# sailab-code/GNN_tf_2.x

Hardware: AMD Instinct MI355X
Metric: node-state-updates/sec (nodes x iters / s), 1M-node synthetic graph (higher is better)
Workload: dtype f32; 1 GPU; synthetic randomGraph-recipe graph, N=1000000 nodes, E=9999690 arcs, state_dim=64, net_state 135->128->128->64 selu+BN, net_output 67->2 softmax+BN, max_iter=30, threshold=0 (all iterations run); the loop-invariant label aggregates (GNN.py:259, :263; 0.2 ms) are kept between Loops until the labels change, see cold_aggregates_ms_per_step; parallelism=single GPU, tile_form=one wave per 32-node tile (k_fused)

## Files before the change

### gnn_tf_2.x_amd/GNN/_engine.py

```python
from __future__ import annotations

import ctypes as C
import os

import numpy as np

_HERE = os.path.dirname(os.path.abspath(__file__))
LIB_PATH = os.environ.get('GNN_HIP_LIBRARY') or os.path.join(_HERE, 'libgnn_hip.so')

ACT_CODES = {'linear': 0, None: 0, 'relu': 1, 'selu': 2, 'elu': 3, 'tanh': 4, 'sigmoid': 5, 'softmax': 6}

EXPORTS = ['gnn_last_error', 'gnn_version', 'gnn_device_count', 'gnn_device_synchronize', 'gnn_graph_create', 'gnn_graph_create_from_arcs',
           'gnn_graph_derive', 'gnn_graph_derive_edge', 'gnn_graph_set_arc_order', 'gnn_graph_update_labels', 'gnn_graph_get_nodes', 'gnn_graph_dims', 'gnn_graph_destroy',
           'gnn_mlp_create', 'gnn_mlp_set_weights', 'gnn_mlp_get_weights', 'gnn_mlp_reset_optimizer', 'gnn_mlp_forward', 'gnn_mlp_destroy', 'gnn_loop_create',
           'gnn_loop_set_state0', 'gnn_loop_run', 'gnn_loop_get_state', 'gnn_loop_get_output', 'gnn_loop_readout', 'gnn_loop_set_edge_readout', 'gnn_loop_train_step',
           'gnn_loop_train_forward', 'gnn_loop_train_backward', 'gnn_loop_arm_optimizer', 'gnn_loop_optimizer_step', 'gnn_loop_update_moving_statistics', 'gnn_loss_grad',
           'gnn_loss_grad_ex', 'gnn_loop_set_loss_params', 'gnn_train_forms', 'gnn_loop_train_forms', 'gnn_loop_train_mask', 'gnn_fused_net_form', 'gnn_small_form',
           'gnn_loop_set_train_persistent', 'gnn_train_persistent_form', 'gnn_loop_train_info',
           'gnn_mlp_set_regularizers', 'gnn_loop_set_clipping', 'gnn_loop_grad_sqnorm', 'gnn_loop_optimizer_step_scaled',
           'gnn_counters_get', 'gnn_lgnn_run', 'gnn_loop_run_many', 'gnn_loop_set_impl', 'gnn_loop_gate_info', 'gnn_loop_set_pieces', 'gnn_loop_range_info', 'gnn_split_f16_exponent', 'gnn_split_f16', 'gnn_loop_set_persistent', 'gnn_loop_set_tile_form', 'gnn_loop_set_gather_form', 'gnn_gather_program_build', 'gnn_graph_gather_program_info', 'gnn_loop_drop_cached_aggregates', 'gnn_loop_set_profiling', 'gnn_loop_get_timing', 'gnn_loop_get_exchange_timing', 'gnn_loop_destroy', 'gnn_shard_range',
           'gnn_comm_unique_id', 'gnn_comm_create', 'gnn_comm_allreduce_max', 'gnn_comm_destroy', 'gnn_halo_plan', 'gnn_graph_create_halo',
           'gnn_comm_create_loopback', 'gnn_graph_set_full_adjacency', 'gnn_loop_set_slice_exchange', 'gnn_loop_run_group', 'gnn_loop_readout_group', 'gnn_graph_update_labels_group']

_lib = None


class EngineError(RuntimeError):
    pass


def lib():
    global _lib
    if _lib is None:
        if not os.path.exists(LIB_PATH):
            raise EngineError(f'{LIB_PATH} is missing: build it with `python -c "import __graft_entry__ as g; g.build()"` '
                              f'or `make -C gnn_tf_2.x_amd/csrc`')
        _lib = C.CDLL(LIB_PATH)
        _lib.gnn_last_error.restype = C.c_char_p
        for name in EXPORTS:
            if name != 'gnn_last_error':
                getattr(_lib, name).restype = C.c_int
    return _lib


def loss_grad(loss_kind: int, targets, out, sample_weights, label_smoothing: float = 0.0, huber_delta: float = 1.0):
    t, o, w = _f32(targets), _f32(out), _f32(sample_weights)
    if t.shape != o.shape or w.shape != (o.shape[0],): raise ValueError(f'targets {t.shape}, outputs {o.shape}, weights {w.shape} do not match')
    d = np.zeros_like(o)
    loss = C.c_double()
    _check(lib().gnn_loss_grad_ex(C.c_int(loss_kind), C.c_int64(o.shape[0]), C.c_int(o.shape[1]), _fp(t), _fp(o), _fp(w), C.c_double(label_smoothing),
                                  C.c_double(huber_delta), C.byref(loss), _fp(d)))
    return float(loss.value), d


FORM_NAMES = {0: 'per_op', 1: 'mlp_fwd', 2: 'wide', 3: 'chain3', 4: 'wgrad_bf', 5: 'wgrad_f32'}


def _forms_dict(out):
    names = [FORM_NAMES[int(v)] for v in out[3:]]
    return dict(forward=names[0::3], backward=names[1::3], wgrad=names[2::3], build_input=bool(out[1]), sweep_rows=int(out[2]))


def train_forms(dims, activations, rates=None, n_rows=0, producer_dropout=True) -> dict:
    L = len(dims) - 1
    if L < 1 or len(activations) != L: raise ValueError('dims needs one entry more than activations')
    d = np.ascontiguousarray(dims, np.int32)
    a = np.asarray([ACT_CODES[x] for x in activations], np.int32)
    r = _f32(rates if rates is not None else np.zeros(L + 1), (L + 1,))
    out = np.zeros(3 + 3 * L, np.int32)
    _check(lib().gnn_train_forms(C.c_int(L), _ip(d), _ip(a), _fp(r), C.c_int64(int(n_rows)), C.c_int(bool(producer_dropout)), _ip(out)))
    return _forms_dict(out)


ACT_NAMES = {v: k for k, v in ACT_CODES.items() if k is not None}


def fused_net_form(dims, activations, nlc=0) -> dict:
    L = len(dims) - 1
    if L < 1 or len(activations) != L: raise ValueError('dims needs one entry more than activations')
    d = np.ascontiguousarray(dims, np.int32)
    a = np.asarray([ACT_CODES[x] for x in activations], np.int32)
    out = np.zeros(6, np.int32)
    _check(lib().gnn_fused_net_form(C.c_int(L), _ip(d), _ip(a), C.c_int(int(nlc)), _ip(out)))
    if not out[0]: return dict(covered=False, hidden=None, last=None, NT=0, NTL=0, mixed=False)
    return dict(covered=True, hidden=ACT_NAMES[int(out[1])], last=ACT_NAMES[int(out[2])], NT=int(out[3]), NTL=int(out[4]), mixed=bool(out[5]))


def small_form(dims, activations, n_rows, nlc=0) -> dict:
    L = len(dims) - 1
    if L < 1 or len(activations) != L: raise ValueError('dims needs one entry more than activations')
    d = np.ascontiguousarray(dims, np.int32)
    a = np.asarray([ACT_CODES[x] for x in activations], np.int32)
    out = np.zeros(3, np.int32)
    _check(lib().gnn_small_form(C.c_int(L), _ip(d), _ip(a), C.c_int(int(nlc)), C.c_int64(int(n_rows)), _ip(out)))
    return dict(persistent=bool(out[0]), tile=int(out[0]), wide=bool(out[1]), steps=int(out[2]))


TRAIN_PERSISTENT_MAX_BYTES = 256 << 20


def train_persistent_form(dims, activations, n_rows, max_iter, rates=None) -> dict:
    L = len(dims) - 1
    if L < 1 or len(activations) != L: raise ValueError('dims needs one entry more than activations')
    d = np.ascontiguousarray(dims, np.int32)
    a = np.asarray([ACT_CODES[x] for x in activations], np.int32)
    r = _f32(rates if rates is not None else np.zeros(L + 1), (L + 1,))
    out = np.zeros(5, np.int32)
    _check(lib().gnn_train_persistent_form(C.c_int(L), _ip(d), _ip(a), _fp(r), C.c_int64(int(n_rows)), C.c_int(int(max_iter)), _ip(out)))
    return dict(persistent=bool(out[0]), workgroups=int(out[1]), rows=int(out[2]), lds=int(out[3]), body_bytes=int(out[4]))


def split_f16(values, exponent=None):
    v = np.ascontiguousarray(values, np.float32).ravel()
    if exponent is None:
        exponent = int(lib().gnn_split_f16_exponent(C.c_float(float(np.max(np.abs(v))) if v.size else 0.0)))
    p0, p1 = np.empty(v.size, np.uint16), np.empty(v.size, np.uint16)
    lib().gnn_split_f16(v.ctypes.data_as(C.c_void_p), C.c_int(v.size), C.c_int(int(exponent)), p0.ctypes.data_as(C.c_void_p), p1.ctypes.data_as(C.c_void_p))
    return p0.view(np.float16), p1.view(np.float16), int(exponent)


def _check(rc: int):
    if rc == 0:
        return
    msg = lib().gnn_last_error().decode(errors='replace')
    if rc == -1:
        raise ValueError(msg)
    if rc == -5:
        raise NotImplementedError(msg)
    raise EngineError(f'[gnn_status {rc}] {msg}')


def _f32(a, shape=None):
    a = np.ascontiguousarray(a, dtype=np.float32)
    if shape is not None and a.shape != tuple(shape):
        raise ValueError(f'expected shape {tuple(shape)}, got {a.shape}')
    return a


def _fp(a):
    return a.ctypes.data_as(C.POINTER(C.c_float)) if a is not None else None


def _ip(a):
    return a.ctypes.data_as(C.POINTER(C.c_int32)) if a is not None else None


def device_count() -> int:
    n = C.c_int(0)
    _check(lib().gnn_device_count(C.byref(n)))
    return n.value


def require_device(device: int = 0) -> None:
    n = device_count()
    if n <= device:
        raise EngineError(f'no HIP device {device} visible ({n} found): this engine only runs on MI355X (gfx950)')


def shard_range(n_nodes: int, rank: int, world: int) -> tuple[int, int]:
    b, n = C.c_int64(0), C.c_int64(0)
    _check(lib().gnn_shard_range(C.c_int64(n_nodes), C.c_int(rank), C.c_int(world), C.byref(b), C.byref(n)))
    return b.value, n.value


def gather_program(indptr, adj_src, adj_w):
    indptr = np.ascontiguousarray(indptr, dtype=np.int32)
    adj_src = np.ascontiguousarray(adj_src, dtype=np.int32)
    adj_w = _f32(adj_w)
    n_rows = indptr.size - 1
    hdr = np.zeros((n_rows // 32, 2), np.int32)
    nb = C.c_int64(0)
    _check(lib().gnn_gather_program_build(C.c_int64(n_rows), _ip(indptr), _ip(adj_src), _fp(adj_w), _ip(hdr), None, C.byref(nb)))
    ent = np.zeros((nb.value, 64, 2), np.int32)
    _check(lib().gnn_gather_program_build(C.c_int64(n_rows), _ip(indptr), _ip(adj_src), _fp(adj_w), None, _ip(ent), C.byref(nb)))
    return hdr, ent.view(np.uint32)


def halo_plan(n_nodes: int, world: int, indptr, adj_src):
    indptr = np.ascontiguousarray(indptr, dtype=np.int32)
    adj_src = np.ascontiguousarray(adj_src, dtype=np.int32)
    slot = np.empty(n_nodes, np.int32)
    counts = np.zeros(world, np.int64)
    block = C.c_int64(0)
    _check(lib().gnn_halo_plan(C.c_int64(n_nodes), C.c_int(world), _ip(indptr), _ip(adj_src), _ip(slot),
                               counts.ctypes.data_as(C.POINTER(C.c_int64)), C.byref(block)))
    return slot, counts, int(block.value)


def shard_halo(n_nodes: int, rank: int, world: int, indptr, adj_src, nodes, plan=None):
    slot, counts, block = plan if plan is not None else halo_plan(n_nodes, world, indptr, adj_src)
    rb, nr = shard_range(n_nodes, rank, world)
    shard = ((n_nodes + world - 1) // world + 31) // 32 * 32
    indptr = np.asarray(indptr)
    e0, e1 = int(indptr[rb]), int(indptr[rb + nr])
    src = np.asarray(adj_src)[e0:e1].astype(np.int64)
    owner = src // shard
    mine = owner == rank
    if np.any(~mine & (slot[src] < 0)):
        raise ValueError('halo plan does not cover a remote source')
    remapped = np.where(mine, src - rb, shard + owner * block + slot[src]).astype(np.int32)
    nodes = np.asarray(nodes, np.float32)
    rep = np.zeros((shard + world * block, nodes.shape[1]), np.float32)
    rep[:nr] = nodes[rb:rb + nr]
    for q in range(world):
        qb, qn = shard_range(n_nodes, q, world)
        ids = qb + np.nonzero(slot[qb:qb + qn] >= 0)[0]
        rep[shard + q * block: shard + q * block + len(ids)] = nodes[ids]
    send = np.nonzero(slot[rb:rb + nr] >= 0)[0].astype(np.int32)
    return dict(block=block, send_rows=send, adj_src=remapped, nodes=rep, row_begin=rb, n_rows=nr, e0=e0, e1=e1)


def shard_csr(n_nodes: int, rank: int, world: int, indptr, *per_entry_arrays):
    rb, nr = shard_range(n_nodes, rank, world)
    indptr = np.asarray(indptr)
    e0, e1 = int(indptr[rb]), int(indptr[rb + nr])
    return (rb, nr, (indptr[rb:rb + nr + 1] - e0).astype(np.int32)) + tuple(np.asarray(a)[e0:e1] for a in per_entry_arrays)


class Graph:

    def __init__(self, n_nodes, indptr, adj_src, adj_w, arc_w, arc_labels, nodes, mask, row_begin=0, device=0, _handle=None):
        self._h = C.c_void_p()
        if _handle is not None:
            self._h = _handle
            return
        require_device(device)
        indptr = np.ascontiguousarray(indptr, dtype=np.int32)
        adj_src = np.ascontiguousarray(adj_src, dtype=np.int32)
        adj_w, arc_w = _f32(adj_w), _f32(arc_w)
        arc_labels, nodes = _f32(arc_labels), _f32(nodes)
        mask = np.ascontiguousarray(mask, dtype=np.uint8)
        n_rows, n_arcs = len(indptr) - 1, len(adj_src)
        if arc_labels.ndim != 2 or arc_labels.shape[0] != n_arcs or nodes.ndim != 2 or nodes.shape[0] != n_nodes:
            raise ValueError('arc_labels must be [n_arcs, AL] and nodes [n_nodes, NL]')
        if len(adj_w) != n_arcs or len(arc_w) != n_arcs or len(mask) != n_rows:
            raise ValueError('inconsistent array lengths')
        _check(lib().gnn_graph_create(C.c_int64(n_nodes), C.c_int64(row_begin), C.c_int64(n_rows), C.c_int64(n_arcs),
                                      _ip(indptr), _ip(adj_src), _fp(adj_w), _fp(arc_w), _fp(arc_labels),
                                      C.c_int(arc_labels.shape[1]), _fp(nodes), C.c_int(nodes.shape[1]),
                                      mask.ctypes.data_as(C.POINTER(C.c_uint8)), C.c_int(device), C.byref(self._h)))

    @classmethod
    def halo(cls, n_nodes_global, rank, world, block, send_rows, indptr, adj_src_replica, adj_w, arc_w, arc_labels, nodes_replica, mask, device=0):
        require_device(device)
        indptr = np.ascontiguousarray(indptr, dtype=np.int32)
        adj = np.ascontiguousarray(adj_src_replica, dtype=np.int32)
        send = np.ascontiguousarray(send_rows, dtype=np.int32)
        adj_w, arc_w, arc_labels, nodes_replica = _f32(adj_w), _f32(arc_w), _f32(arc_labels), _f32(nodes_replica)
        mask = np.ascontiguousarray(mask, dtype=np.uint8)
        if len(adj_w) != len(adj) or len(arc_w) != len(adj) or arc_labels.shape[0] != len(adj) or len(mask) != len(indptr) - 1:
            raise ValueError('inconsistent array lengths')
        h = C.c_void_p()
        _check(lib().gnn_graph_create_halo(C.c_int64(n_nodes_global), C.c_int(rank), C.c_int(world), C.c_int64(block), C.c_int64(len(send)), _ip(send),
                                           C.c_int64(len(adj)), _ip(indptr), _ip(adj), _fp(adj_w), _fp(arc_w), _fp(arc_labels), C.c_int(arc_labels.shape[1]),
                                           _fp(nodes_replica), C.c_int(nodes_replica.shape[1]), mask.ctypes.data_as(C.POINTER(C.c_uint8)), C.c_int(device), C.byref(h)))
        return cls(None, None, None, None, None, None, None, None, _handle=h)

    @classmethod
    def from_arcs(cls, n_nodes, arc_src, arc_dst, arc_labels, aggregation_mode, nodes, mask, device=0):
        require_device(device)
        modes = {'sum': 0, 'normalized': 1, 'average': 2}
        if aggregation_mode not in modes: raise ValueError('ERROR: Unknown aggregation mode')
        arc_src = np.ascontiguousarray(arc_src, dtype=np.int32)
        arc_dst = np.ascontiguousarray(arc_dst, dtype=np.int32)
        arc_labels, nodes = _f32(arc_labels), _f32(nodes)
        mask = np.ascontiguousarray(mask, dtype=np.uint8)
        e = len(arc_src)
        if len(arc_dst) != e or arc_labels.shape[0] != e or nodes.shape[0] != n_nodes or len(mask) != n_nodes:
            raise ValueError('inconsistent array lengths')
        indptr, adj_src, arc_id = np.zeros(n_nodes + 1, np.int32), np.zeros(e, np.int32), np.zeros(e, np.int32)
        adj_w, arc_w = np.zeros(e, np.float32), np.zeros(e, np.float32)
        h = C.c_void_p()
        _check(lib().gnn_graph_create_from_arcs(C.c_int64(n_nodes), C.c_int64(e), _ip(arc_src), _ip(arc_dst), _fp(arc_labels),
                                                C.c_int(arc_labels.shape[1]), C.c_int(modes[aggregation_mode]), _fp(nodes), C.c_int(nodes.shape[1]),
                                                mask.ctypes.data_as(C.POINTER(C.c_uint8)), C.c_int(device), C.byref(h), _ip(indptr), _ip(adj_src),
                                                _fp(adj_w), _ip(arc_id), _fp(arc_w)))
        return cls(None, None, None, None, None, None, None, None, _handle=h), indptr, adj_src, adj_w, arc_id, arc_w

    def dims(self):
        n, r, e, m = C.c_int64(), C.c_int64(), C.c_int64(), C.c_int64()
        nl, al = C.c_int(), C.c_int()
        _check(lib().gnn_graph_dims(self._h, C.byref(n), C.byref(r), C.byref(e), C.byref(nl), C.byref(al), C.byref(m)))
        return dict(n_nodes=n.value, n_rows=r.value, n_arcs=e.value, NL=nl.value, AL=al.value, n_masked=m.value)

    def derive(self, extra: int) -> 'Graph':
        h = C.c_void_p()
        _check(lib().gnn_graph_derive(self._h, C.c_int(extra), C.byref(h)))
        d = Graph(None, None, None, None, None, None, None, None, _handle=h)
        d._base = self
        return d

    def derive_edge(self, extra_nodes: int, extra_arcs: int) -> 'Graph':
        h = C.c_void_p()
        _check(lib().gnn_graph_derive_edge(self._h, C.c_int(extra_nodes), C.c_int(extra_arcs), C.byref(h)))
        d = Graph(None, None, None, None, None, None, None, None, _handle=h)
        d._base = self
        return d

    def gather_program_info(self) -> dict:
        t, b, n, ms = C.c_int64(0), C.c_int64(0), C.c_int64(0), C.c_float(0)
        _check(lib().gnn_graph_gather_program_info(self._h, C.byref(t), C.byref(b), C.byref(n), C.byref(ms)))
        return dict(tiles=t.value, batches=b.value, bytes=n.value, build_ms=ms.value)

    def set_arc_order(self, arc_id, arc_labels_orig) -> None:
        arc_id = np.ascontiguousarray(arc_id, dtype=np.int32)
        _check(lib().gnn_graph_set_arc_order(self._h, _ip(arc_id), _fp(_f32(arc_labels_orig))))

    def update_labels(self, base: 'Graph', loop: 'Loop', get_state: bool, get_output: bool) -> None:
        _check(lib().gnn_graph_update_labels(self._h, base._h, loop._h, C.c_int(bool(get_state)), C.c_int(bool(get_output))))

    def set_full_adjacency(self, n_global: int, indptr, adj_src, adj_w):
        ip, src, w = np.ascontiguousarray(indptr, np.int32), np.ascontiguousarray(adj_src, np.int32), _f32(adj_w)
        _check(lib().gnn_graph_set_full_adjacency(self._h, C.c_int64(n_global), _ip(ip), _ip(src), _fp(w)))

    @staticmethod
    def update_labels_group(dsts, bases, loops, get_state: bool, get_output: bool) -> None:
        n = len(loops)
        arr = lambda xs: (C.c_void_p * n)(*[x._h for x in xs])
        _check(lib().gnn_graph_update_labels_group(arr(dsts), arr(bases), arr(loops), C.c_int(n), C.c_int(bool(get_state)), C.c_int(bool(get_output))))

    def nodes(self) -> np.ndarray:
        d = self.dims()
        out = np.empty((d['n_nodes'], d['NL']), dtype=np.float32)
        _check(lib().gnn_graph_get_nodes(self._h, _fp(out)))
        return out

    def close(self):
        if self._h:
            lib().gnn_graph_destroy(self._h)
            self._h = C.c_void_p()

    def __del__(self):
        try:
            self.close()
        except Exception:
            pass


class Mlp:

    def __init__(self, weights, activations, batch_normalization, bn_eps=1e-3, device=0):
        require_device(device)
        self._h = C.c_void_p()
        self.n = len(activations)
        self.activations = list(activations)
        self.batch_normalization = bool(batch_normalization)
        for a in activations:
            if a not in ACT_CODES:
                raise ValueError(f'unsupported activation {a!r}')
        w, b, bn = self._pack(weights)
        self.dims = np.array([w[0].shape[0]] + [x.shape[1] for x in w], dtype=np.int32)
        acts = np.array([ACT_CODES[a] for a in activations], dtype=np.int32)
        wp = (C.POINTER(C.c_float) * self.n)(*[_fp(x) for x in w])
        bp = (C.POINTER(C.c_float) * self.n)(*[_fp(x) for x in b])
        _check(lib().gnn_mlp_create(C.c_int(self.n), _ip(self.dims), _ip(acts), wp, bp, _fp(bn), C.c_float(bn_eps),
                                    C.c_int(device), C.byref(self._h)))

    def _pack(self, weights):
        n = self.n
        if len(weights) != 2 * n + (4 if self.batch_normalization else 0):
            raise ValueError(f'expected {2 * n + (4 if self.batch_normalization else 0)} weight arrays, got {len(weights)}')
        w = [_f32(weights[2 * l]) for l in range(n)]
        b = [_f32(weights[2 * l + 1]) for l in range(n)]
        for l in range(n):
            if w[l].ndim != 2 or b[l].shape != (w[l].shape[1],) or (l and w[l].shape[0] != w[l - 1].shape[1]):
                raise ValueError(f'layer {l}: inconsistent weight shapes')
        bn = None
        if self.batch_normalization:
            bn = np.ascontiguousarray(np.concatenate([_f32(a).ravel() for a in weights[2 * n:]]))
            if bn.size != 4 * w[-1].shape[1]:
                raise ValueError('BatchNormalization arrays must each have the output width')
        return w, b, bn

    def set_weights(self, weights):
        w, b, bn = self._pack(weights)
        if [x.shape for x in w] != [(int(self.dims[l]), int(self.dims[l + 1])) for l in range(self.n)]:
            raise ValueError('weight shapes differ from the ones this MLP was created with')
        wp = (C.POINTER(C.c_float) * self.n)(*[_fp(x) for x in w])
        bp = (C.POINTER(C.c_float) * self.n)(*[_fp(x) for x in b])
        _check(lib().gnn_mlp_set_weights(self._h, wp, bp, _fp(bn)))

    def get_weights(self):
        w = [np.empty((int(self.dims[l]), int(self.dims[l + 1])), np.float32) for l in range(self.n)]
        b = [np.empty((int(self.dims[l + 1]),), np.float32) for l in range(self.n)]
        f = int(self.dims[-1])
# ... 235 lines not shown
        gs = np.zeros(sum(int(np.prod(x)) for x in shp_s), np.float32)
        go = np.zeros(sum(int(np.prod(x)) for x in shp_o), np.float32)
        bns = np.zeros((max(1, kk), 2, int(net_state.dims[-1])), np.float32)
        bno = np.zeros((2, int(net_output.dims[-1])), np.float32)
        d_out = _f32(d_out_nodes)
        if d_out.shape != (self.n_masked, self.T): raise ValueError(f'd_out_nodes shape {d_out.shape} != {(self.n_masked, self.T)}')
        dse = None
        if d_state_extra is not None:
            dse = _f32(d_state_extra)
            if dse.shape != (self.n_rows, self.Ds): raise ValueError(f'd_state_extra shape {dse.shape} != {(self.n_rows, self.Ds)}')
        dims = self.graph.dims()
        dn = np.zeros((self.n_rows, dims['NL']), np.float32) if want_d_nodes else None
        da = np.zeros((dims['n_arcs'], dims['AL']), np.float32) if want_d_arcs else None
        _check(lib().gnn_loop_train_backward(self._h, _fp(d_out), _fp(dse), _fp(gs), _fp(go), _fp(bns), _fp(bno), _fp(dn), _fp(da)))

        def split(flat, shp):
            out, off = [], 0
            for x in shp:
                cnt = int(np.prod(x))
                out.append(flat[off:off + cnt].reshape(x).copy())
                off += cnt
            return out

        return dict(grads_state=split(gs, shp_s), grads_output=split(go, shp_o), bn_batch_state=bns[:kk], bn_batch_output=bno, d_nodes=dn, d_arcs=da)

    def train_forms(self, net: int = 0) -> dict:
        out = np.zeros(3 + 3 * self._keep[1 + net].n, np.int32)
        _check(lib().gnn_loop_train_forms(self._h, C.c_int(net), _ip(out)))
        return _forms_dict(out)

    def train_mask(self, net: int, body: int, pos: int) -> np.ndarray:
        count = C.c_int64()
        _check(lib().gnn_loop_train_mask(self._h, C.c_int(net), C.c_int(body), C.c_int(pos), None, C.byref(count)))
        width = int(self._keep[1 + net].dims[pos])
        out = np.zeros(count.value, np.uint8)
        _check(lib().gnn_loop_train_mask(self._h, C.c_int(net), C.c_int(body), C.c_int(pos), out.ctypes.data_as(C.POINTER(C.c_uint8)), C.byref(count)))
        return out.reshape(-1, width).astype(bool)

    def set_impl(self, impl: int) -> int:
        used = C.c_int(0)
        _check(lib().gnn_loop_set_impl(self._h, C.c_int(impl), C.byref(used)))
        return used.value

    def gate_info(self) -> tuple:
        a, b = C.c_int(0), C.c_int(0)
        _check(lib().gnn_loop_gate_info(self._h, C.byref(a), C.byref(b)))
        return bool(a.value), int(b.value)

    def set_pieces(self, pieces: int) -> int:
        used = C.c_int(0)
        _check(lib().gnn_loop_set_pieces(self._h, C.c_int(int(pieces)), C.byref(used)))
        return used.value

    def range_info(self) -> tuple:
        a, b = C.c_int(0), C.c_int(0)
        _check(lib().gnn_loop_range_info(self._h, C.byref(a), C.byref(b)))
        return bool(a.value), int(b.value)

    def set_persistent(self, enable: bool) -> bool:
        used = C.c_int(0)
        _check(lib().gnn_loop_set_persistent(self._h, C.c_int(bool(enable)), C.byref(used)))
        return bool(used.value)

    def set_train_persistent(self, enable: bool) -> bool:
        used = C.c_int(0)
        _check(lib().gnn_loop_set_train_persistent(self._h, C.c_int(bool(enable)), C.byref(used)))
        return bool(used.value)

    def train_info(self) -> dict:
        out = np.zeros(4, np.int32)
        _check(lib().gnn_loop_train_info(self._h, _ip(out)))
        return dict(persistent=bool(out[0]), workgroups=int(out[1]), barriers_per_body=int(out[2]), timeouts=int(out[3]))

    def set_tile_form(self, form: int) -> int:
        used = C.c_int(0)
        _check(lib().gnn_loop_set_tile_form(self._h, C.c_int(int(form)), C.byref(used)))
        return used.value

    def set_gather_form(self, form: int) -> int:
        used = C.c_int(0)
        _check(lib().gnn_loop_set_gather_form(self._h, C.c_int(int(form)), C.byref(used)))
        return used.value

    def counters(self) -> dict:
        b, f, it, tot, avg = C.c_double(), C.c_double(), C.c_int(), C.c_float(), C.c_float()
        _check(lib().gnn_counters_get(self._h, C.byref(b), C.byref(f), C.byref(it), C.byref(tot), C.byref(avg)))
        return dict(bytes_per_iteration=b.value, flops_per_iteration=f.value, iterations=it.value, total_ms=tot.value, avg_iteration_ms=avg.value)

    @staticmethod
    def lgnn_run(loops, graphs, get_state: bool, get_output: bool) -> list:
        n = len(loops)
        ks = (C.c_float * n)()
        _check(lib().gnn_lgnn_run((C.c_void_p * n)(*[x._h for x in loops]), (C.c_void_p * n)(*[x._h for x in graphs]), C.c_int(n),
                                  C.c_int(bool(get_state)), C.c_int(bool(get_output)), ks))
        return [float(k) for k in ks]

    def drop_cached_aggregates(self):
        _check(lib().gnn_loop_drop_cached_aggregates(self._h))

    def set_profiling(self, on: bool):
        _check(lib().gnn_loop_set_profiling(self._h, C.c_int(bool(on))))

    def run(self, training: bool = False) -> float:
        k = C.c_float(0)
        _check(lib().gnn_loop_run(self._h, C.c_int(bool(training)), C.byref(k)))
        return float(k.value)

    @staticmethod
    def run_many(loops) -> list:
        n = len(loops)
        hs = (C.c_void_p * n)(*[l._h for l in loops])
        ks = (C.c_float * n)()
        _check(lib().gnn_loop_run_many(hs, C.c_int(n), ks))
        return [float(x) for x in ks]

    @staticmethod
    def run_group(loops) -> float:
        n = len(loops)
        hs = (C.c_void_p * n)(*[l._h for l in loops])
        k = C.c_float(0)
        _check(lib().gnn_loop_run_group(hs, C.c_int(n), C.byref(k)))
        return float(k.value)

    @staticmethod
    def readout_group(loops, ng_indptr, ng_node, ng_w) -> np.ndarray:
        n = len(loops)
        hs = (C.c_void_p * n)(*[l._h for l in loops])
        ng_indptr = np.ascontiguousarray(ng_indptr, dtype=np.int32)
        ng_node = np.ascontiguousarray(ng_node, dtype=np.int32)
        ng_w = _f32(ng_w)
        g = len(ng_indptr) - 1
        out = np.empty((g, loops[0].T), dtype=np.float32)
        _check(lib().gnn_loop_readout_group(hs, C.c_int(n), C.c_int(g), _ip(ng_indptr), _ip(ng_node), _fp(ng_w), _fp(out)))
        return out

    def timing(self):
        tot, avg, n = C.c_float(), C.c_float(), C.c_int()
        _check(lib().gnn_loop_get_timing(self._h, C.byref(tot), C.byref(avg), C.byref(n)))
        gap = C.c_float()
        _check(lib().gnn_loop_get_exchange_timing(self._h, C.byref(gap)))
        return dict(total_ms=tot.value, avg_iter_ms=avg.value, n_iter_timed=n.value, avg_between_bodies_ms=gap.value)

    def state(self) -> np.ndarray:
        out = np.empty((self.n_rows, self.Ds), dtype=np.float32)
        _check(lib().gnn_loop_get_state(self._h, _fp(out)))
        return out

    def output(self) -> np.ndarray:
        out = np.empty((self.n_masked, self.T), dtype=np.float32)
        m = C.c_int64(0)
        _check(lib().gnn_loop_get_output(self._h, _fp(out), C.byref(m)))
        return out

    def readout(self, ng_indptr, ng_node, ng_w) -> np.ndarray:
        ng_indptr = np.ascontiguousarray(ng_indptr, dtype=np.int32)
        ng_node = np.ascontiguousarray(ng_node, dtype=np.int32)
        ng_w = _f32(ng_w)
        g = len(ng_indptr) - 1
        out = np.empty((g, self.T), dtype=np.float32)
        _check(lib().gnn_loop_readout(self._h, C.c_int(g), _ip(ng_indptr), _ip(ng_node), _fp(ng_w), _fp(out)))
        return out

    def close(self):
        if self._h:
            lib().gnn_loop_destroy(self._h)
            self._h = C.c_void_p()
# ... 7 lines not shown
```

### gnn_tf_2.x_amd/csrc/gnn_build.hip

```cpp
#include <hipcub/hipcub.hpp>
#include <string.h>

#include <algorithm>
#include <chrono>
#include <new>
#include <vector>

#include "gnn_common.h"
#include "gnn_fused.h"

namespace {

inline unsigned cdiv(int64_t a, int64_t b) { return (unsigned)((a + b - 1) / b); }

__global__ void k_keys(int64_t e, const int32_t *src, const int32_t *dst, unsigned long long *key, int32_t *id, int32_t *indeg)
{
    const int64_t a = (int64_t)blockIdx.x * blockDim.x + threadIdx.x;
    if (a >= e) return;
    key[a] = ((unsigned long long)(uint32_t)dst[a] << 32) | (uint32_t)src[a];
    id[a] = (int32_t)a;
    atomicAdd(indeg + dst[a], 1);
}

__global__ void k_values(int64_t e, const int32_t *dst, const int32_t *indeg, int mode, float *w)
// ... 152 lines not shown
        if (adj_w_out) HIPCHK_G(hipMemcpy(adj_w_out, sh->adj_w, sizeof(float) * E, hipMemcpyDeviceToHost));
        if (arc_id_out) HIPCHK_G(hipMemcpy(arc_id_out, d_perm2, sizeof(int32_t) * E, hipMemcpyDeviceToHost));
        if (arc_w_out) HIPCHK_G(hipMemcpy(arc_w_out, sh->arc_w, sizeof(float) * E, hipMemcpyDeviceToHost));
    }
    *out = g;
    return GNN_OK;
#undef HIPCHK_G
}

namespace {

void gather_program_split(const int (&slots)[32], int (&start)[5], int &longest)
{
    int lo = 0, hi = 0;
    for (int r = 0; r < 32; ++r) { lo = std::max(lo, slots[r]); hi += slots[r]; }
    auto groups_needed = [&](int cap) {
        int n = 1, fill = 0;
        for (int r = 0; r < 32; ++r) {
            if (fill + slots[r] > cap) { ++n; fill = 0; }
            fill += slots[r];
        }
        return n;
    };
    while (lo < hi) {
        const int mid = lo + (hi - lo) / 2;
        if (groups_needed(mid) <= 4) hi = mid; else lo = mid + 1;
    }
    int g = 0, fill = 0;
    start[0] = 0;
    for (int r = 0; r < 32; ++r) {
        if (fill + slots[r] > lo) { start[++g] = r; fill = 0; }
        fill += slots[r];
    }
    while (g < 4) start[++g] = 32;
    longest = lo;
}

}

extern "C" int gnn_gather_program_build(int64_t n_rows, const int32_t *indptr, const int32_t *adj_src, const float *adj_w, int32_t *hdr,
                                        int32_t *ent, int64_t *n_batches)
{
    ARGCHK(n_rows >= 0 && indptr && n_batches, "n_rows / indptr / n_batches are required");
    const int64_t tiles = n_rows / 32;
    ARGCHK(indptr[tiles * 32] == 0 || (adj_src && adj_w), "arc arrays are required");
    int64_t batch = 0;
    for (int64_t t = 0; t < tiles; ++t) {
        const int32_t *ip = indptr + t * 32;
        int slots[32], start[5], longest = 0;
        for (int r = 0; r < 32; ++r) {
            ARGCHK(ip[r + 1] >= ip[r], "indptr not monotone at row %lld", (long long)(t * 32 + r));
            slots[r] = std::max(1, ip[r + 1] - ip[r]);
        }
        gather_program_split(slots, start, longest);
        const int nb = (longest + 15) / 16;
        ARGCHK(batch + nb < ((int64_t)1 << 31) / 64, "gather program too large");
        if (hdr) { hdr[2 * t] = (int32_t)batch; hdr[2 * t + 1] = nb; }
        if (ent) {
            for (int g = 0; g < 4; ++g) {
                int s = 0;
                auto put = [&](uint32_t word, float w) {
                    int32_t *e = ent + (((batch + s / 16) * 64 + 16 * g + s % 16) * 2);
                    memcpy(e, &word, 4);
                    memcpy(e + 1, &w, 4);
                    ++s;
                };
                for (int r = start[g]; r < start[g + 1]; ++r) {
                    if (ip[r + 1] == ip[r]) put(GNN_GP_NOROW | GNN_GP_ROW_END | (uint32_t)r, 0.0f);
                    for (int32_t e = ip[r]; e < ip[r + 1]; ++e) {
                        if (adj_src[e] < 0 || adj_src[e] >= (1 << 23))
                            return gnn_fail(GNN_ERR_UNSUPPORTED, "adj_src[%d]=%d does not fit a gather-program source word", e, adj_src[e]);
                        put((uint32_t)adj_src[e] << 8 | (e + 1 == ip[r + 1] ? GNN_GP_ROW_END : 0u) | (uint32_t)r, adj_w[e]);
                    }
                }
                while (s < 16 * nb) put(GNN_GP_NOROW, 0.0f);
            }
        }
        batch += nb;
    }
    *n_batches = batch;
    return GNN_OK;
}

int gnn_gather_program_ensure(const gnn_graph *g)
{
    gnn_graph_shared *sh = g->sh;
    if (sh->gp_tried) return GNN_OK;
    sh->gp_tried = true;
    const int64_t tiles = g->n_rows / 32, rem = g->n_rows % 32;
    if (tiles == 0) return GNN_OK;
    int dev_before = -1;
    if (hipGetDevice(&dev_before) != hipSuccess || hipSetDevice(g->device) != hipSuccess) { (void)hipGetLastError(); return GNN_OK; }
    const auto t0 = std::chrono::steady_clock::now();
    int32_t *d_hdr = nullptr, *d_ent = nullptr;
    int64_t batches = 0, last_batches = 0;
    int32_t last_hdr[2] = {0, 0};
    bool ok = false;
    try {
        std::vector<int32_t> indptr((size_t)g->n_rows + 1), hdr((size_t)tiles * 2), src, ent;
        std::vector<float> w;
        ok = hipMemcpy(indptr.data(), sh->indptr, sizeof(int32_t) * indptr.size(), hipMemcpyDeviceToHost) == hipSuccess;
        const size_t E = ok ? (size_t)indptr.back() : 0;
        if (rem) indptr.resize((size_t)(tiles + 1) * 32 + 1, indptr.back());
        src.resize(E); w.resize(E);
        ok = ok && (E == 0 || (hipMemcpy(src.data(), sh->adj_src, sizeof(int32_t) * E, hipMemcpyDeviceToHost) == hipSuccess &&
                               hipMemcpy(w.data(), sh->adj_w, sizeof(float) * E, hipMemcpyDeviceToHost) == hipSuccess));
        for (size_t e = 0; ok && e < E; ++e) ok = src[e] >= 0 && src[e] < (1 << 23);
        const int32_t *last_ip = indptr.data() + tiles * 32;
        ok = ok && gnn_gather_program_build(tiles * 32, indptr.data(), src.data(), w.data(), hdr.data(), nullptr, &batches) == GNN_OK;
        if (ok && rem) ok = gnn_gather_program_build(32, last_ip, src.data(), w.data(), last_hdr, nullptr, &last_batches) == GNN_OK;
        ok = ok && batches + last_batches < ((int64_t)1 << 31) / 64;
        if (ok) {
            ent.resize((size_t)(batches + last_batches) * 128);
            ok = gnn_gather_program_build(tiles * 32, indptr.data(), src.data(), w.data(), nullptr, ent.data(), &batches) == GNN_OK;
            if (ok && rem) ok = gnn_gather_program_build(32, last_ip, src.data(), w.data(), nullptr, ent.data() + (size_t)batches * 128, &last_batches) == GNN_OK;
        }
        ok = ok && gnn_dev_malloc((void **)&d_hdr, sizeof(int32_t) * hdr.size()) == hipSuccess &&
             gnn_dev_malloc((void **)&d_ent, sizeof(int32_t) * ent.size()) == hipSuccess &&
             hipMemcpy(d_hdr, hdr.data(), sizeof(int32_t) * hdr.size(), hipMemcpyHostToDevice) == hipSuccess &&
             hipMemcpy(d_ent, ent.data(), sizeof(int32_t) * ent.size(), hipMemcpyHostToDevice) == hipSuccess;
    } catch (const std::bad_alloc &) { ok = false; }
    if (ok) {
        sh->gp_hdr = d_hdr; sh->gp_ent = d_ent; sh->gp_tiles = tiles; sh->gp_batches = batches + last_batches;
        sh->gp_rows = g->n_rows; sh->gp_last_first = (int32_t)batches; sh->gp_last_nb = (int32_t)last_batches;
        sh->gp_build_ms = std::chrono::duration<float, std::milli>(std::chrono::steady_clock::now() - t0).count();
    } else {
        (void)hipFree(d_hdr); (void)hipFree(d_ent);
        (void)hipGetLastError();
    }
    (void)hipSetDevice(dev_before);
    return GNN_OK;
}

extern "C" int gnn_graph_gather_program_info(const gnn_graph *g, int64_t *tiles, int64_t *batches, int64_t *bytes, float *build_ms)
{
    ARGCHK(g, "graph is NULL");
    const gnn_graph_shared *sh = g->sh;
    const bool have = sh->gp_ent != nullptr;
    if (tiles) *tiles = have ? sh->gp_tiles : 0;
    if (batches) *batches = have ? sh->gp_batches : 0;
    if (bytes) *bytes = have ? sh->gp_tiles * 8 + sh->gp_batches * 512 : 0;
    if (build_ms) *build_ms = have ? sh->gp_build_ms : 0.0f;
    return GNN_OK;
}
```

### gnn_tf_2.x_amd/csrc/gnn_common.h

```cpp
#pragma once
#include <hip/hip_runtime.h>
#include <stdint.h>
#include <string>
#include <vector>

#include "gnn_hip.h"
#include "gnn_fused.h"

int gnn_fail(int code, const char *fmt, ...);

hipError_t gnn_dev_malloc(void **p, size_t bytes);
bool gnn_poison_enabled();

inline hipError_t gnn_raise_dynamic_lds(const void *const *kernels, int n, size_t bytes, bool (&raised)[64])
{
    int dev = 0;
    hipError_t e = hipGetDevice(&dev);
    if (e != hipSuccess) return e;
    const bool listed = dev >= 0 && dev < 64;
    if (listed && raised[dev]) return hipSuccess;
    for (int i = 0; i < n && e == hipSuccess; ++i) e = hipFuncSetAttribute(kernels[i], hipFuncAttributeMaxDynamicSharedMemorySize, (int)bytes);
    if (listed && e == hipSuccess) raised[dev] = true;
    return e;
}
// ... 53 lines not shown
#define GNN_FLAG_WORDS (GNN_FLAG_SLOTS * GNN_FLAG_STRIDE)
#define GNN_BODY_CHUNK 16
#define GNN_BODY_LOOKAHEAD 4

__device__ __forceinline__ bool gnn_gate_open(const int *gate, int world)
{
    if (!gate) return true;
    int any = 0;
    for (int p = 0; p < world * GNN_FLAG_SLOTS; ++p) any |= gate[p * GNN_FLAG_STRIDE];
    return any != 0;
}

__device__ __forceinline__ bool gnn_gate_open_block(const int *gate, int world)
{
    if (!gate) return true;
    __shared__ int gate_any;
    if (threadIdx.x == 0) gate_any = 0;
    __syncthreads();
    int any = 0;
    for (int p = threadIdx.x; p < world * GNN_FLAG_SLOTS; p += blockDim.x) any |= gate[p * GNN_FLAG_STRIDE];
    if (any) gate_any = 1;
    __syncthreads();
    return gate_any != 0;
}

__device__ __forceinline__ void gnn_flag_raise(int *flag_rank_base)
{
    int *w = flag_rank_base + (blockIdx.x & (GNN_FLAG_SLOTS - 1)) * GNN_FLAG_STRIDE;
    if (__hip_atomic_load(w, __ATOMIC_RELAXED, __HIP_MEMORY_SCOPE_AGENT) == 0) atomicOr(w, 1);
}

#define GNN_BAND_ABS 1e-5f
#define GNN_BAND_REL 1e-3f
__device__ __forceinline__ bool gnn_gate_borderline(float root, float rhs, float band) { return band > 0.0f && __builtin_fabsf(root - rhs) <= band; }
struct GnnFlagPeek { int c0, c1, c2; };
__device__ __forceinline__ GnnFlagPeek gnn_flag_peek(int *flag_rank_base)
{
    int *w = flag_rank_base + (blockIdx.x & (GNN_FLAG_SLOTS - 1)) * GNN_FLAG_STRIDE;
    GnnFlagPeek p;
    p.c0 = __hip_atomic_load(w, __ATOMIC_RELAXED, __HIP_MEMORY_SCOPE_AGENT);
    p.c1 = __hip_atomic_load(w + 1, __ATOMIC_RELAXED, __HIP_MEMORY_SCOPE_AGENT);
    p.c2 = __hip_atomic_load(w + 2, __ATOMIC_RELAXED, __HIP_MEMORY_SCOPE_AGENT);
    return p;
}
__device__ __forceinline__ void gnn_flag_raise_peeked(int *flag_rank_base, const GnnFlagPeek &p, bool moved, bool robust, bool border)
{
    int *w = flag_rank_base + (blockIdx.x & (GNN_FLAG_SLOTS - 1)) * GNN_FLAG_STRIDE;
    if (moved && p.c0 == 0) atomicOr(w, 1);
    if (robust && p.c1 == 0) atomicOr(w + 1, 1);
    if (border && p.c2 == 0) atomicOr(w + 2, 1);
}

__device__ __forceinline__ void gnn_flag_raise_certified(int *flag_rank_base, bool moved, bool robust, bool border)
{
    int *w = flag_rank_base + (blockIdx.x & (GNN_FLAG_SLOTS - 1)) * GNN_FLAG_STRIDE;
    if (!(moved || border)) return;
    const int c0 = __hip_atomic_load(w, __ATOMIC_RELAXED, __HIP_MEMORY_SCOPE_AGENT);
    const int c1 = __hip_atomic_load(w + 1, __ATOMIC_RELAXED, __HIP_MEMORY_SCOPE_AGENT);
    const int c2 = __hip_atomic_load(w + 2, __ATOMIC_RELAXED, __HIP_MEMORY_SCOPE_AGENT);
    if (moved && c0 == 0) atomicOr(w, 1);
    if (robust && c1 == 0) atomicOr(w + 1, 1);
    if (border && c2 == 0) atomicOr(w + 2, 1);
}

struct gnn_graph_shared {
    int refs = 1;
    int32_t *indptr = nullptr, *adj_src = nullptr, *masked_rows = nullptr;
    float *adj_w = nullptr, *arc_w = nullptr, *arc_labels = nullptr;
    uint8_t *mask = nullptr;
    int max_degree = 0;
    int32_t *src_indptr = nullptr, *src_dst = nullptr;
    float *src_w = nullptr;
    int32_t *arc_id = nullptr;
    float *arc_labels_orig = nullptr;
    int32_t *full_indptr = nullptr, *full_src = nullptr;
    float *full_w = nullptr;
    int64_t full_rows = 0;
    int32_t *gp_hdr = nullptr, *gp_ent = nullptr;
    int64_t gp_tiles = 0, gp_batches = 0;
    int64_t gp_rows = 0;
    int32_t gp_last_first = 0, gp_last_nb = 0;
    bool gp_tried = false;
    float gp_build_ms = 0.0f;
};

struct gnn_graph {
    int device = 0;
    int64_t N = 0, N_global = 0, row_begin = 0, own_off = 0, n_rows = 0, E = 0, n_masked = 0;
    int NL = 0, AL = 0;
    int halo_world = 0, halo_rank = 0;
    int64_t halo_block = 0, halo_count = 0;
    int32_t *halo_send = nullptr;
    bool halo_send_owned = true;
    int64_t nodes_rows = 0;
    gnn_graph_shared *sh = nullptr;
    float *nodes = nullptr;
    int base_NL = 0;
    float *arc_labels_own = nullptr, *arc_labels_orig_own = nullptr;
    int base_AL = 0;
    uint64_t label_version = 1;
    hipEvent_t ready = nullptr;
};

inline const float *gnn_graph_arc_labels(const gnn_graph *g) { return g->arc_labels_own ? g->arc_labels_own : g->sh->arc_labels; }

struct gnn_mlp {
    int device = 0;
    int n_layers = 0;
    std::vector<int> dims, acts;
    std::vector<float *> W, b;
    float *slab = nullptr;
    size_t slab_floats = 0;
    float *bn_scale = nullptr, *bn_shift = nullptr;
    float *bn_raw = nullptr;
    float *opt_a = nullptr, *opt_b = nullptr;
    float *opt_c = nullptr;
    int opt_kind = -1;
    std::vector<double> reg_l1, reg_l2;
    bool has_bn = false;
    float eps = 1e-3f;
    float *packed = nullptr;
    size_t packed_floats = 0;
    int *packed_split = nullptr;
    size_t packed_split_dwords = 0;
    int split_exp[3] = {0, 0, 0};
    int pack_nlc = -1;
    bool pack_dirty = true;
    uint64_t version = 0;
};

struct gnn_loop;
struct gnn_comm_group {
    int world = 1, refs = 0;
    hipStream_t stream = nullptr;
    std::vector<gnn_loop *> member;
};

struct gnn_comm {
    int rank = 0, world = 1, device = 0;
    void *nccl = nullptr;
    gnn_comm_group *grp = nullptr;
    hipStream_t stream = nullptr;
    hipStream_t xstream = nullptr;
    double *scratch = nullptr;
    int loops = 0;
    bool closed = false;
};

struct gnn_train_settings {
    struct { bool armed = false; int kind = 0; float h[4] = {0, 0, 0, 0}; bool mean = false; float mom_s = 0.99f, mom_o = 0.99f; } opt;
    struct { float value = 0.0f; double norm = 0.0, global = 0.0; } clip;
    struct { double smoothing = 0.0, delta = 1.0; } loss;
    struct { bool allowed = false, failed = false; int timeouts = 0; } persistent;
    int k_hint = 0;
};
#define GNN_INTERNAL __attribute__((visibility("hidden")))
struct GNN_INTERNAL gnn_train_ctx;
struct GNN_INTERNAL gnn_train_arena;

struct gnn_loop {
    gnn_graph *g = nullptr;
    gnn_mlp *st = nullptr, *ou = nullptr;
    gnn_comm *comm = nullptr;
    int device = 0, rank = 0, world = 1;
    int D = 0, Ds = 0, NLc = 0, in_s = 0, wf = 0, T = 0, max_iter = 0;
    float thr = 0.f;
    int64_t shard_rows = 0, N_pad = 0, own_off = 0;
    hipStream_t stream = nullptr;
    float *state[2] = {nullptr, nullptr};
    float *state_init = nullptr;
    bool init_in_place = false;
    float *inp = nullptr;
    float *inv = nullptr;
    uint64_t inv_version = 0;
    bool inv_zeroed = false;
    float *tmp[2] = {nullptr, nullptr};
    float *feats = nullptr, *out = nullptr, *otmp[2] = {nullptr, nullptr};
    int *flags = nullptr;
    int *tile_ctr = nullptr;
    int *kfinal_dev = nullptr, *kfinal_host = nullptr;
    int certified_reruns = 0;
    bool last_run_rerun = false;
    int pieces = 2;
    int range_reruns = 0;
    bool last_run_range_rerun = false;
    bool small_words_clean = false;
    unsigned small_runs = 0;
    float *small_xs = nullptr;
    size_t small_xs_floats = 0;
    bool small_disabled = false;
    int kfinal = -1;
    bool have_state0 = false, ran = false;
    bool graph_ready_seen = false;
    int impl_req = 1;
    int tile_form = 0;
    int gather_form = 0;
    LoopForm form;
    int32_t *ng_ip = nullptr, *ng_node = nullptr;
    float *ng_w = nullptr, *ng_out = nullptr, *ng_part = nullptr;
    std::vector<int32_t> ng_key;
    std::vector<float> ng_w_host;
    float *ng_host = nullptr;
    int ng_G = 0, ng_host_floats = 0;
    bool ng_inlaunch = false;
    uint64_t out_runs = 0, ng_inlaunch_run = 0;
    bool edge_mode = false, edge_expected = false;
    int32_t *edge_dst = nullptr, *edge_rows = nullptr;
    float *edge_labels = nullptr;
    int64_t n_edge_masked = 0;
    int32_t *edge_inc_ptr = nullptr, *edge_inc = nullptr;
    int *gate_host = nullptr;
    hipEvent_t ev_gate = nullptr;
    bool profiling = false;
    std::vector<hipEvent_t> ev;
    hipEvent_t ev_total[2] = {nullptr, nullptr};
    float total_ms = 0.f, avg_iter_ms = 0.f;
    float avg_gap_ms = 0.f;
    int n_iter_timed = 0;
    bool slice_mode = false;
    int Cs = 0;
    float *sl_send = nullptr;
    float *sl_state = nullptr;
    float *sl_agg = nullptr;
    float *sl_recv = nullptr;
    bool sl_pipeline = true;
    std::vector<hipEvent_t> sl_ev;
    hipEvent_t sl_done = nullptr;
    float *agg_own = nullptr;
    gnn_train_ctx *train_ctx = nullptr;
    gnn_train_arena *train_arena = nullptr;
    gnn_train_settings train;
};

inline bool gnn_loop_ng_folded(const gnn_loop *l) { return l->ng_inlaunch && l->ng_inlaunch_run == l->out_runs; }

int gnn_graph_wait_ready(const gnn_graph *g, hipStream_t st);
int gnn_launch_spmm(hipStream_t st, int64_t n_rows, const int32_t *indptr, const int32_t *idx, const float *w, const float *X,
                    int width, int64_t ldx, float *out, int64_t ldo, const int *gate, int world);
int gnn_launch_dense(hipStream_t st, int64_t n, int n_in, int n_out, const float *X, int64_t ldx, const float *W, const float *b,
                     int act, float *Y, int64_t ldy);
int gnn_launch_check(hipStream_t st, int64_t n_rows, int d, const float *s, const float *so, float thr, int *flag_rank_base);
int gnn_comm_allgather32(gnn_comm *c, const void *send, void *recv, size_t count, hipStream_t st);
int gnn_launch_feats_edge(hipStream_t st, const gnn_loop *l, const float *state, float *feats);
int gnn_launch_copy_cols(hipStream_t st, int64_t n_rows, int w, const float *src, int64_t lds_, float *dst, int64_t ldd, const int *gate, int world);
int gnn_mlp_refresh_bn(gnn_mlp *m, hipStream_t st);
void gnn_train_ctx_free(gnn_loop *l);
void gnn_train_arena_free(gnn_loop *l);

int gnn_loop_decide_form(gnn_loop *l);
inline int gnn_loop_impl_used(const gnn_loop *l) { return l->form.path == GNN_PATH_UNFUSED ? 0 : (l->form.split ? 2 : 1); }
int gnn_gather_program_ensure(const gnn_graph *g);
int gnn_fused_prepare(gnn_loop *l);
int gnn_fused_pack(gnn_mlp *m, int nlc);
int gnn_fused_iteration(gnn_loop *l, int k);
int gnn_small_run(gnn_loop *l);
void gnn_fused_release(gnn_mlp *m);
```

### gnn_tf_2.x_amd/csrc/gnn_fused.h

```cpp
#pragma once
#include <hip/hip_runtime.h>
#include <stdint.h>

constexpr int GNN_FUSED_MAXL = 3;
constexpr int GNN_FUSED_WAVES = 8;
constexpr int GNN_FUSED_THREADS = 64 * GNN_FUSED_WAVES;
#define GNN_F16_EX 4
#define GNN_F16_LIMIT 65504.0f
#define GNN_GP_ROW_MASK 31u
#define GNN_GP_ROW_END 32u
#define GNN_GP_NOROW 0xfffffe00u
constexpr int GNN_ACTL_FROM_ARGS = -1;

struct GnnFusedArgs {
    int64_t n_rows, row_begin;
    const int32_t *indptr, *adj_src;
    const float *adj_w;
    const float *inv;
    const float *state_cur;
    float *state_nxt;
    int64_t state_bytes;
    int Ds, NLc, AL, IW, in_s, c_aggs, KP, lpr, lpr_log2, vec, kk0;
    const float *Wp[GNN_FUSED_MAXL];
    const float *bias[GNN_FUSED_MAXL];
    const float *bn_scale, *bn_shift;
    float thr;
    const int *gate;
    int *flag_out;
    int world;
    int certify;
    int *tile_ctr;
    int wstride;
    int stagger;
    const int *Ws[GNN_FUSED_MAXL];
    int chunks0;
    int pieces;
    float bsc[GNN_FUSED_MAXL], usc[GNN_FUSED_MAXL];
    const int *Ws_base;
    int ws_bytes, ws_off[GNN_FUSED_MAXL];
    int tile_base;
    int full_tiles;
    int variant;
    const float *agg_in;
    const int32_t *gp_hdr, *gp_ent;
    int gp_tiles, gp_last_first, gp_last_nb;
    int threads;
    int single_ticket;
    unsigned long long *stamps;
    int lds_floats;
    int act_last;
};

struct GnnSmallCtl {
    float *state0, *state1;
    const float *init;
    int *kfinal;
    int *flags;
    int *host_result;
    float *xs;
    int DP;
    int rnd;
    const float *Wraw[GNN_FUSED_MAXL];
    int din[GNN_FUSED_MAXL], dout[GNN_FUSED_MAXL];
    int KP16;
    int *zero_words;
    int n_words;
    int max_iter;
    float *out;
    const uint8_t *mask;
    const int32_t *mask_pos;
    const float *nodes_own;
    const float *ow, *ob, *obn_scale, *obn_shift;
    int NL, NLc, T, oact;
    const int32_t *ng_ip, *ng_node;
    const float *ng_w;
    float *ng_host;
    int G, ro_word;
    int ecache;
};

struct FusedPlan {
    int layers = 0, NT = 0, NTL = 0, KP = 0, kk0 = 0;
    int act = 0, act_last = 0;
    int pad = 0, KPs = 0;
    int nt[GNN_FUSED_MAXL] = {0, 0, 0};
    int kk[GNN_FUSED_MAXL] = {0, 0, 0};
    size_t w_off[GNN_FUSED_MAXL] = {0, 0, 0}, b_off[GNN_FUSED_MAXL] = {0, 0, 0}, bn_off = 0, total = 0;
    int chunks[GNN_FUSED_MAXL] = {0, 0, 0};
    size_t s_off[GNN_FUSED_MAXL] = {0, 0, 0}, h_off[GNN_FUSED_MAXL] = {0, 0, 0}, s_total = 0;
};

enum GnnLoopPath { GNN_PATH_UNFUSED = 0, GNN_PATH_BODIES = 1, GNN_PATH_PERSISTENT = 2 };
enum GnnBodyKernel { GNN_BODY_GENERIC = 0, GNN_BODY_FULL_TILE = 1, GNN_BODY_PAIR = 2 };
struct LoopForm {
    int path = GNN_PATH_UNFUSED;
    int kernel = GNN_BODY_GENERIC;
    bool split = false;
    int pieces = 3;
    bool program = false;
    FusedPlan plan;
    unsigned grid = 0;
    size_t lds = 0;
    GnnFusedArgs args;
    int small_tile = 0, kk_small = 0, s0 = 0;
    bool small_wide = false;
    bool fold_output = false, fold_readout = false;
    GnnSmallCtl ctl;
};

constexpr int GNN_SMALL_ECACHE = 1024;
constexpr int GNN_SMALL16_HP = 36;
constexpr int GNN_SMALL16W_HP = 66;
template <int ROWS, bool WIDE = false>
struct GnnSmallLds {
    static_assert(ROWS == 16 || ROWS == 32, "16- or 32-node tiles");
    static_assert(!WIDE || ROWS == 16, "the wide form works on 16-node tiles");
    static constexpr int H = 0;
    static constexpr int IPT = ROWS == 16 ? 16 * (WIDE ? GNN_SMALL16W_HP : GNN_SMALL16_HP) : 32;
    static constexpr int EP = IPT + ROWS + 4;
    static constexpr int HBW = WIDE ? 64 : 32;
    static constexpr int HB = EP + 96;
    static constexpr int HW = HB + 2 * HBW;
    static constexpr int SCR = HW + 544;
    static constexpr int LABELS = 32 * ROWS;
    static constexpr int EC_SRC = SCR + 2 * LABELS;
    static constexpr int EC_W = EC_SRC + GNN_SMALL_ECACHE;
    static constexpr int END = EC_W + GNN_SMALL_ECACHE + 4;
    static constexpr size_t bytes(int KP) { return sizeof(float) * ((size_t)ROWS * KP + END); }
};

template <int... V> struct GnnSteps { static constexpr int values[] = {V...}; };
using GnnSmallKK0 = GnnSteps<8, 12, 16, 24, 32, 36, 40, 48>;
using GnnSmall16S0 = GnnSteps<4, 8, 12, 16, 20, 24>;

bool gnn_small_launch(int layers, int act, int kk0, const GnnFusedArgs &a, const GnnSmallCtl &c, unsigned grid, size_t lds_bytes,
                      hipStream_t st);
bool gnn_small16_launch(int layers, int act, int s0, const GnnFusedArgs &a, const GnnSmallCtl &c, unsigned grid, size_t lds_bytes, hipStream_t st);
bool gnn_small_launch_mixed(int layers, int act, int kk0, const GnnFusedArgs &a, const GnnSmallCtl &c, unsigned grid, size_t lds_bytes,
                            hipStream_t st);
bool gnn_small16_launch_mixed(int layers, int act, int s0, const GnnFusedArgs &a, const GnnSmallCtl &c, unsigned grid, size_t lds_bytes, hipStream_t st);
bool gnn_small16w_launch(int layers, int act, int s0, const GnnFusedArgs &a, const GnnSmallCtl &c, unsigned grid, size_t lds_bytes, hipStream_t st);
bool gnn_small16w_launch_mixed(int layers, int act, int s0, const GnnFusedArgs &a, const GnnSmallCtl &c, unsigned grid, size_t lds_bytes, hipStream_t st);

bool gnn_fused_launch_l1(int act, int nt, int ntl, const GnnFusedArgs &a, unsigned grid, size_t lds_bytes, hipStream_t st);
bool gnn_fused_launch_s1(int act, int nt, int ntl, const GnnFusedArgs &a, unsigned grid, size_t lds_bytes, hipStream_t st);
bool gnn_fused_launch_s2(int act, int nt, int ntl, const GnnFusedArgs &a, unsigned grid, size_t lds_bytes, hipStream_t st);
bool gnn_fused_launch_s3(int act, int nt, int ntl, const GnnFusedArgs &a, unsigned grid, size_t lds_bytes, hipStream_t st);
bool gnn_fused_launch_p2(int act, const GnnFusedArgs &a, unsigned grid, size_t lds_bytes, hipStream_t st);
bool gnn_fused_launch_p3(int act, const GnnFusedArgs &a, unsigned grid, size_t lds_bytes, hipStream_t st);
bool gnn_fused_launch_l2(int act, int nt, int ntl, const GnnFusedArgs &a, unsigned grid, size_t lds_bytes, hipStream_t st);
bool gnn_fused_launch_l3(int act, int nt, int ntl, const GnnFusedArgs &a, unsigned grid, size_t lds_bytes, hipStream_t st);
bool gnn_fused_launch_ml2(int act, int nt, int ntl, const GnnFusedArgs &a, unsigned grid, size_t lds_bytes, hipStream_t st);
bool gnn_fused_launch_ml3(int act, int nt, int ntl, const GnnFusedArgs &a, unsigned grid, size_t lds_bytes, hipStream_t st);
bool gnn_fused_launch_ms2(int act, int nt, int ntl, const GnnFusedArgs &a, unsigned grid, size_t lds_bytes, hipStream_t st);
bool gnn_fused_launch_ms3(int act, int nt, int ntl, const GnnFusedArgs &a, unsigned grid, size_t lds_bytes, hipStream_t st);
```

### gnn_tf_2.x_amd/csrc/gnn_fused.hip

```cpp
#include <stdio.h>
#include <stdlib.h>
#include <string.h>

#include <algorithm>
#include <cmath>
#include <vector>

#include "gnn_engine.h"
#include "gnn_fused.h"

namespace {

constexpr int MAXL = GNN_FUSED_MAXL;
constexpr int K_GROUP = 12;
constexpr int K_SLACK = 8;

constexpr int GNN_FUSED_VARIANT_DEFAULT = 1;
constexpr int GNN_FUSED_SPREAD_DEFAULT = 8;
constexpr int GNN_FUSED_SPREAD_SMALL_DEFAULT = 6;
#ifndef GNN_GATHER_FORM_DEFAULT
#define GNN_GATHER_FORM_DEFAULT 2
#endif
constexpr int S_SLACK = 2;

int round_tiles(int width) { return width <= 32 ? 1 : (width <= 64 ? 2 : 4); }

bool make_plan(const gnn_mlp *m, int nlc, FusedPlan &p)
{
    if (m->n_layers < 1 || m->n_layers > MAXL) return false;
    p.layers = m->n_layers;
    p.act_last = m->acts[m->n_layers - 1];
    p.act = m->n_layers > 1 ? m->acts[0] : p.act_last;
    int hid = 0;
    for (int l = 0; l < m->n_layers; ++l) {
        if (m->acts[l] < GNN_ACT_LINEAR || m->acts[l] >= GNN_ACT_SOFTMAX) return false;
        if (l < m->n_layers - 1 && m->acts[l] != p.act) return false;
        if (m->dims[l + 1] > 128) return false;
        if (l < m->n_layers - 1) hid = std::max(hid, m->dims[l + 1]);
    }
    p.NTL = round_tiles(m->dims.back());
    if (p.layers == 1) {
        p.NT = p.NTL;
    } else {
        p.NT = std::max(round_tiles(hid), p.NTL);
        if (p.NT > 1 && p.NTL == 1) p.NTL = 2;
    }
    p.kk0 = ((m->dims[0] + 1) / 2 + K_GROUP - 1) / K_GROUP * K_GROUP;
    p.KP = std::max(2 * p.kk0, (m->dims[0] + 15) / 16 * 16) + 1;
    size_t off = 0;
    for (int l = 0; l < p.layers; ++l) {
        p.nt[l] = l == p.layers - 1 ? p.NTL : p.NT;
        p.kk[l] = l == 0 ? p.kk0 : 16 * p.NT;
        p.w_off[l] = off;
        off += (size_t)(p.kk[l] + (l == 0 ? K_SLACK : 0)) * 64 * p.nt[l];
    }
    for (int l = 0; l < p.layers; ++l) { p.b_off[l] = off; off += 32 * (size_t)p.nt[l]; }
    p.bn_off = off;
    off += 2 * 32 * (size_t)p.NTL;
    p.total = off;
    const int ds = m->dims.back();
    p.pad = ds == 64 ? (4 - (ds + nlc) % 4) % 4 : 0;
    p.KPs = p.KP;
    if (ds == 64) {
        p.KPs = (std::max(2 * p.kk0, (m->dims[0] + p.pad + 15) / 16 * 16) + 3) / 4 * 4;
        if ((p.KPs / 4) % 2 == 0) p.KPs += 4;
    }
    size_t soff = 0;
    for (int l = 0; l < p.layers; ++l) {
        p.chunks[l] = l == 0 ? (m->dims[0] + p.pad + 15) / 16 : 2 * p.NT;
        p.s_off[l] = soff;
        soff += (size_t)(p.chunks[l] + (l == 0 ? S_SLACK : 0)) * p.nt[l] * 3 * 256;
    }
    for (int l = 0; l < p.layers; ++l) {
        p.h_off[l] = soff;
        soff += (size_t)(p.chunks[l] + (l == 0 ? S_SLACK : 0)) * p.nt[l] * 2 * 256;
    }
    p.s_total = soff;
    return true;
}

size_t lds_bytes(const FusedPlan &p)
{
    return (size_t)GNN_FUSED_WAVES * 32 * std::max(p.KP, p.KPs) * sizeof(float) + 128 + GNN_FUSED_WAVES * 36 * sizeof(int) + (3 + 2) * 32 * 4 * sizeof(float) + 16;
}

constexpr int PAIR_CH0 = 9;
bool pair_covers(const FusedPlan &p, int ds)
{
    return ds == 64 && p.NTL == 2 && p.NT == 4 && (p.layers == 2 || p.layers == 3) && p.chunks[0] == PAIR_CH0 && p.act_last == p.act;
}
int pair_xs(const FusedPlan &p)
{
    int xs = 16 * p.chunks[0] - 64 + 4;
    if ((xs / 4) % 2 == 0) xs += 4;
    return xs;
}
size_t pair_lds_bytes(const FusedPlan &p)
{
    return sizeof(float) * ((size_t)4 * (32 * pair_xs(p) + p.chunks[0] * 768) + 16 + GNN_FUSED_WAVES * 20 + 3 * 32 * 2 + 2 * 32 * 4) + 128;
}
struct SmallForm {
    int tile = 0;
    bool wide = false;
    int steps = 0;
// ... 243 lines not shown
    a.KP = split ? p.KPs : p.KP; a.kk0 = p.kk0;
    a.vec = (l->Ds % 4 == 0) ? 4 : 1;
    int lpr = 1, lg = 0;
    while ((lpr * a.vec < l->Ds || lpr < 2) && lpr < 64) { lpr <<= 1; ++lg; }
    a.lpr = lpr; a.lpr_log2 = lg;
    for (int i = 0; i < p.layers; ++i) {
        a.Wp[i] = m->packed + p.w_off[i];
        a.bias[i] = m->packed + p.b_off[i];
    }
    for (int i = 0; i < p.layers; ++i) a.Ws[i] = m->packed_split + p.s_off[i];
    a.chunks0 = p.chunks[0];
    a.Ws_base = m->packed_split;
    a.ws_bytes = (int)(p.s_total * sizeof(uint32_t));
    a.pieces = l->pieces == 2 ? 2 : 3;
    for (int i = 0; i < p.layers; ++i) {
        a.ws_off[i] = (int)((a.pieces == 2 ? p.h_off[i] : p.s_off[i]) * sizeof(uint32_t));
        const int e = a.pieces == 2 ? m->split_exp[i] + GNN_F16_EX : 0;
        a.bsc[i] = std::ldexp(1.0f, e);
        a.usc[i] = std::ldexp(1.0f, -e);
    }
    a.variant = GNN_FUSED_VARIANT_DEFAULT;
    a.bn_scale = m->has_bn ? m->packed + p.bn_off : nullptr;
    a.bn_shift = m->has_bn ? m->packed + p.bn_off + 32 * p.NTL : nullptr;
    a.thr = l->thr;
    a.world = l->world;
    a.certify = split ? 1 : 0;
    a.agg_in = l->slice_mode ? l->agg_own : nullptr;
    a.wstride = 1;
    a.act_last = p.act_last;
}

static void body_args(const gnn_loop *l, int k, GnnFusedArgs &a)
{
    const int cur = k & 1, P = l->world;
    a.state_cur = gnn_loop_state_after(l, k, 0);
    a.state_nxt = l->state[cur ^ 1] + (size_t)l->own_off * l->Ds;
    a.gate = l->flags + (size_t)k * P * GNN_FLAG_WORDS;
    a.flag_out = l->flags + ((size_t)(k + 1) * P + l->rank) * GNN_FLAG_WORDS;
    a.tile_ctr = l->tile_ctr + k;
}

static void decide_bodies(const gnn_loop *l, LoopForm &f, int n_cu)
{
    const gnn_graph *g = l->g;
    const FusedPlan &p = f.plan;
    GnnFusedArgs &a = f.args;
    fill_args(l, p, f.split, a);
    const size_t n_tiles = (size_t)((g->n_rows + 31) / 32);
#ifdef GNN_DIAG
    static const int variant_env = getenv("GNN_FUSED_VARIANT") ? atoi(getenv("GNN_FUSED_VARIANT")) : GNN_FUSED_VARIANT_DEFAULT;
    a.variant = variant_env;
    static const int debug = getenv("GNN_FUSED_DEBUG") ? atoi(getenv("GNN_FUSED_DEBUG")) : 0;
    a.wstride = (debug & 1) ? 0 : 1;
#endif
    const unsigned grid = (unsigned)std::min<size_t>((size_t)n_cu, n_tiles);
    int stagger_rounds = GNN_FUSED_SPREAD_DEFAULT;
#ifdef GNN_DIAG
    static const int stagger_env = getenv("GNN_FUSED_STAGGER") ? atoi(getenv("GNN_FUSED_STAGGER")) : GNN_FUSED_SPREAD_DEFAULT;
    stagger_rounds = stagger_env;
#endif
    a.stagger = n_tiles >= (size_t)4 * GNN_FUSED_WAVES * grid ? stagger_rounds : (n_tiles > (size_t)GNN_FUSED_WAVES * grid ? GNN_FUSED_SPREAD_SMALL_DEFAULT : 0);
#ifdef GNN_DIAG
    static const int stagger_small = getenv("GNN_FUSED_STAGGER_SMALL") ? atoi(getenv("GNN_FUSED_STAGGER_SMALL")) : 0;
    const bool small_grid = n_tiles > (size_t)GNN_FUSED_WAVES * grid && n_tiles < (size_t)4 * GNN_FUSED_WAVES * grid;
    if (small_grid && stagger_small > 0) { a.stagger = stagger_small; a.variant |= 4; }
    static const int spread_small = getenv("GNN_FUSED_SPREAD_SMALL") ? atoi(getenv("GNN_FUSED_SPREAD_SMALL")) : -1;
    if (small_grid && spread_small >= 0) a.stagger = spread_small;
#endif
    a.single_ticket = n_tiles <= (size_t)GNN_FUSED_WAVES * grid ? 1 : 0;
    f.grid = grid;
    f.lds = lds_bytes(p);
    if (f.kernel == GNN_BODY_PAIR) {
        const int64_t n_tiles64 = (int64_t)n_tiles;
        a.KP = pair_xs(p);
        a.full_tiles = 1;
        f.grid = (unsigned)std::min<int64_t>((int64_t)n_cu, (n_tiles64 + 3) / 4);
        a.stagger = n_tiles64 >= (int64_t)4 * 4 * f.grid ? stagger_rounds : (n_tiles64 > (int64_t)4 * f.grid ? GNN_FUSED_SPREAD_SMALL_DEFAULT : 0);
        f.lds = pair_lds_bytes(p);
    } else if (f.kernel == GNN_BODY_FULL_TILE) {
        a.full_tiles = 1;
        if (f.program) {
            a.gp_hdr = g->sh->gp_hdr; a.gp_ent = g->sh->gp_ent; a.gp_tiles = (int)g->sh->gp_tiles;
            a.gp_last_first = g->sh->gp_last_first; a.gp_last_nb = g->sh->gp_last_nb;
        }
    }
    a.lds_floats = gnn_poison_enabled() ? (int)(f.lds / sizeof(float)) : 0;
}

static int decide_persistent(gnn_loop *l, LoopForm &f, const SmallForm &sf)
{
    const gnn_graph *g = l->g;
    const FusedPlan &p = f.plan;
    GnnFusedArgs &a = f.args;
    fill_args(l, p, false, a);
    a.state_cur = l->state[0];
    a.state_nxt = l->state[1] + (size_t)l->own_off * l->Ds;
    GnnSmallCtl &c = f.ctl;
    c.state0 = l->state[0]; c.state1 = l->state[1];
    c.init = l->D ? l->state_init : g->nodes + (size_t)g->own_off * g->NL;
    c.kfinal = l->kfinal_dev;
    c.host_result = l->kfinal_host;
    bool tile16 = sf.tile == 16;
    f.small_wide = sf.wide;
    if (tile16) f.s0 = sf.steps; else f.kk_small = sf.steps;
#ifdef GNN_DIAG
    static const int tile_env = getenv("GNN_SMALL_TILE") ? atoi(getenv("GNN_SMALL_TILE")) : 0;
    if (tile_env == 32 && !sf.wide) {
        tile16 = false;
        f.kk_small = small_form(l->st, p, 16 * 256 + 1).steps;
    }
#endif
    f.small_tile = tile16 ? 16 : 32;
    f.grid = (unsigned)((g->n_rows + f.small_tile - 1) / f.small_tile);
    c.DP = l->Ds <= 16 ? 16 : 32;
    {
        const size_t need = (size_t)2 * f.grid * f.small_tile * c.DP;
        if (l->small_xs_floats < need) {
            if (l->small_xs) (void)hipFree(l->small_xs);
            l->small_xs = nullptr; l->small_xs_floats = 0;
            HIPCHK(gnn_dev_malloc((void **)&l->small_xs, need * sizeof(float)));
            l->small_xs_floats = need;
        }
        c.xs = l->small_xs;
    }
    c.max_iter = l->max_iter;
    c.ecache = GNN_SMALL_ECACHE;
#ifdef GNN_DIAG
    static const int ecache_env = getenv("GNN_SMALL_ECACHE") ? atoi(getenv("GNN_SMALL_ECACHE")) : GNN_SMALL_ECACHE;
    c.ecache = std::min(GNN_SMALL_ECACHE, ecache_env);
#endif
    c.n_words = (int)(((size_t)l->max_iter + 3 + 3) & ~(size_t)3);
    const gnn_mlp *ou = l->ou;
    if (!l->edge_mode && g->n_masked && ou->n_layers == 1 && l->T <= 8 && l->Ds + l->NLc <= 64 && l->Ds <= 32 && g->NL <= 32) {
        c.out = l->out; c.mask = g->sh->mask; c.mask_pos = g->sh->masked_rows + g->n_masked;
        c.nodes_own = g->nodes + (size_t)g->own_off * g->NL;
        c.ow = ou->W[0]; c.ob = ou->b[0];
        c.obn_scale = ou->has_bn ? ou->bn_scale : nullptr; c.obn_shift = ou->has_bn ? ou->bn_shift : nullptr;
        c.NL = g->NL; c.NLc = l->NLc; c.T = l->T; c.oact = ou->acts[0];
        f.fold_output = true;
        if (l->ng_ip && l->ng_G > 0 && g->n_masked == g->n_rows) {
            if (l->ng_host_floats < l->ng_G * l->T) {
                if (l->ng_host) (void)hipHostFree(l->ng_host);
                l->ng_host = nullptr; l->ng_host_floats = 0;
                if (hipHostMalloc((void **)&l->ng_host, sizeof(float) * (size_t)l->ng_G * l->T) == hipSuccess) l->ng_host_floats = l->ng_G * l->T;
            }
            if (l->ng_host) {
                c.ng_ip = l->ng_ip; c.ng_node = l->ng_node; c.ng_w = l->ng_w; c.ng_host = l->ng_host; c.G = l->ng_G; c.ro_word = l->max_iter + 1;
                f.fold_readout = true;
            }
        }
    }
    c.rnd = g->sh->max_degree > 8 ? 8 : 4;
    if (tile16) {
        const gnn_mlp *m = l->st;
        for (int q = 0; q < p.layers; ++q) { c.Wraw[q] = m->W[q]; c.din[q] = m->dims[q]; c.dout[q] = m->dims[q + 1]; }
        c.KP16 = std::max((a.in_s + 3) / 4 * 4, 4 * f.s0);
        if (c.KP16 % 8 == 0) c.KP16 += 4;
        f.lds = sf.wide ? GnnSmallLds<16, true>::bytes(c.KP16) : GnnSmallLds<16>::bytes(c.KP16);
    } else
        f.lds = GnnSmallLds<32>::bytes(p.KP);
    a.lds_floats = gnn_poison_enabled() ? (int)(f.lds / sizeof(float)) : 0;
    return GNN_OK;
}

int gnn_loop_decide_form(gnn_loop *l)
{
    LoopForm &f = l->form;
    f = LoopForm{};
    if (l->impl_req < 1) return GNN_OK;
    HIPCHK(hipSetDevice(l->device));
    if (!gnn_fused_supported(l, f.plan)) return GNN_OK;
    if (l->device < 0 || l->device >= 64) return gnn_fail(GNN_ERR_ARG, "device %d out of range", l->device);
    const gnn_graph *g = l->g;
    const FusedPlan &p = f.plan;
    const int n_cu = device_cus(l->device);
    const int64_t n_tiles = (g->n_rows + 31) / 32;
    f.split = l->impl_req == 2;
    f.pieces = l->pieces == 2 ? 2 : 3;
    const bool pair = f.split && !l->slice_mode && pair_covers(p, l->Ds) && pair_lds_bytes(p) <= 160 * 1024 &&
                      (l->tile_form ? l->tile_form == 2 : n_tiles <= (int64_t)4 * n_cu);
    f.kernel = pair ? GNN_BODY_PAIR : (l->Ds == 64 && p.NTL == 2 ? GNN_BODY_FULL_TILE : GNN_BODY_GENERIC);
    if (f.kernel == GNN_BODY_FULL_TILE && !l->slice_mode && (l->gather_form ? l->gather_form : GNN_GATHER_FORM_DEFAULT) == 2 &&
        gnn_gather_program_ensure(g) == GNN_OK)
        f.program = g->sh->gp_ent != nullptr && g->sh->gp_rows == g->n_rows;
    const SmallForm sf = small_form(l->st, p, g->n_rows);
    const bool persistent = l->world == 1 && !l->small_disabled && !l->profiling && sf.tile != 0;
    f.path = persistent ? GNN_PATH_PERSISTENT : GNN_PATH_BODIES;
    if (!l->inv) HIPCHK(gnn_dev_malloc((void **)&l->inv, inv_floats(l) * sizeof(float)));
    if (persistent) return decide_persistent(l, f, sf);
    decide_bodies(l, f, n_cu);
    return GNN_OK;
}

static bool launch_body(const LoopForm &f, const GnnFusedArgs &a, hipStream_t st)
{
    const FusedPlan &p = f.plan;
    if (p.act_last != p.act) {
        if (f.kernel == GNN_BODY_PAIR || p.layers < 2) return false;
        if (f.split) return p.layers == 2 ? gnn_fused_launch_ms2(p.act, p.NT, p.NTL, a, f.grid, f.lds, st) : gnn_fused_launch_ms3(p.act, p.NT, p.NTL, a, f.grid, f.lds, st);
        return p.layers == 2 ? gnn_fused_launch_ml2(p.act, p.NT, p.NTL, a, f.grid, f.lds, st) : gnn_fused_launch_ml3(p.act, p.NT, p.NTL, a, f.grid, f.lds, st);
    }
    if (f.kernel == GNN_BODY_PAIR)
        return p.layers == 2 ? gnn_fused_launch_p2(p.act, a, f.grid, f.lds, st) : gnn_fused_launch_p3(p.act, a, f.grid, f.lds, st);
    if (f.split) {
        if (p.layers == 1) return gnn_fused_launch_s1(p.act, p.NT, p.NTL, a, f.grid, f.lds, st);
        if (p.layers == 2) return gnn_fused_launch_s2(p.act, p.NT, p.NTL, a, f.grid, f.lds, st);
        return gnn_fused_launch_s3(p.act, p.NT, p.NTL, a, f.grid, f.lds, st);
    }
    if (p.layers == 1) return gnn_fused_launch_l1(p.act, p.NT, p.NTL, a, f.grid, f.lds, st);
    if (p.layers == 2) return gnn_fused_launch_l2(p.act, p.NT, p.NTL, a, f.grid, f.lds, st);
    return gnn_fused_launch_l3(p.act, p.NT, p.NTL, a, f.grid, f.lds, st);
}

int gnn_fused_iteration(gnn_loop *l, int k)
{
    const LoopForm &f = l->form;
    GnnFusedArgs a = f.args;
    body_args(l, k, a);
#ifdef GNN_DIAG
    static const char *stamp_file = getenv("GNN_FUSED_STAMPS");
    static unsigned long long *stamp_buf = nullptr;
    const size_t n_waves = (size_t)((l->g->n_rows + 31) / 32);
    if (stamp_file && k == 1) {
        if (!stamp_buf) HIPCHK(gnn_dev_malloc((void **)&stamp_buf, n_waves * 16 * sizeof(unsigned long long)));
        HIPCHK(hipMemsetAsync(stamp_buf, 0, n_waves * 16 * sizeof(unsigned long long), l->stream));
        a.stamps = stamp_buf;
    }
#endif
    const FusedPlan &p = f.plan;
    if (!launch_body(f, a, l->stream))
        return gnn_fail(GNN_ERR_UNSUPPORTED, "no fused instantiation for %d layers, tiles (%d,%d), activations %d / %d", p.layers, p.NT, p.NTL, p.act, p.act_last);
#ifdef GNN_DIAG
    if (a.stamps) {
        std::vector<unsigned long long> host(n_waves * (f.kernel == GNN_BODY_PAIR ? 16 : 8));
        HIPCHK(hipStreamSynchronize(l->stream));
        HIPCHK(hipMemcpy(host.data(), stamp_buf, host.size() * sizeof(unsigned long long), hipMemcpyDeviceToHost));
        if (FILE *f_ = fopen(stamp_file, "wb")) { fwrite(host.data(), sizeof(unsigned long long), host.size(), f_); fclose(f_); }
    }
#endif
    HIPCHK(hipGetLastError());
    return GNN_OK;
}

int gnn_small_run(gnn_loop *l)
{
    const LoopForm &f = l->form;
    const FusedPlan &p = f.plan;
    GnnFusedArgs a = f.args;
    GnnSmallCtl c = f.ctl;
    const size_t n_words = (size_t)c.n_words;
    l->kfinal_host[1] = 0;
    if (!l->small_words_clean) {
        HIPCHK(hipMemsetAsync(l->flags, 0, sizeof(int) * 2 * n_words, l->stream));
        l->small_words_clean = true;
        l->small_runs = 0;
    }
    c.flags = l->flags + (l->small_runs & 1) * n_words;
    c.zero_words = l->flags + ((l->small_runs & 1) ^ 1) * n_words;
    ++l->small_runs;
    l->ng_inlaunch = f.fold_readout;
    if (f.fold_readout) l->ng_inlaunch_run = l->out_runs;
#ifdef GNN_DIAG
    static const char *small_stamp_file = getenv("GNN_SMALL_STAMPS");
    static unsigned long long *small_stamp_buf = nullptr;
    if (small_stamp_file) {
        if (!small_stamp_buf) HIPCHK(gnn_dev_malloc((void **)&small_stamp_buf, 256 * sizeof(unsigned long long)));
        HIPCHK(hipMemsetAsync(small_stamp_buf, 0, 256 * sizeof(unsigned long long), l->stream));
// ... 26 lines not shown
```

### gnn_tf_2.x_amd/csrc/gnn_fused_kernel.h

```cpp
#pragma once
#include <utility>

#include "gnn_common.h"
#include "gnn_fused.h"

typedef float f32x16 __attribute__((ext_vector_type(16)));

namespace gnn_fused_dev {

#define GNN_GLOBAL __attribute__((address_space(1)))
template <class T>
__device__ __forceinline__ const GNN_GLOBAL T *gptr(const T *p) { return (const GNN_GLOBAL T *)p; }
template <class T>
__device__ __forceinline__ GNN_GLOBAL T *gptr_w(T *p) { return (GNN_GLOBAL T *)p; }
typedef float v4f __attribute__((ext_vector_type(4)));
typedef float v2f __attribute__((ext_vector_type(2)));
typedef int v4i_ __attribute__((ext_vector_type(4)));
__device__ __forceinline__ v4f gload4(const float *p) { return *(const GNN_GLOBAL v4f *)p; }
#ifndef GNN_STORE_AUX
#define GNN_STORE_AUX 2
#endif
__device__ __forceinline__ void gstore_row4(float *base, int64_t off, v4f v)
{
#if GNN_STORE_AUX == 0
// ... 811 lines not shown
    if constexpr (!PADDED) zero_pad_columns(a, X, lane, KP);
    __builtin_amdgcn_fence(__ATOMIC_ACQ_REL, "wavefront");

    int node = grp * 8;
    const int node_end = node + 8;
    const int e_begin = ipt[node], e_end = ipt[node_end];
    int next_end = ipt[node + 1];
    v2f acc01 = {0.f, 0.f}, acc23 = {0.f, 0.f};
    const __amdgpu_buffer_rsrc_t rsrc = __builtin_amdgcn_make_buffer_rsrc(const_cast<float *>(a.state_cur), 0, (int)a.state_bytes, 0x00020000);
    const int voff0 = gl * 16;
    float *xo = X + c_aggs + gl * 4;
#define GNN_ROW_BOUNDARY(e)                                                                     \
    while ((e) >= next_end) {                                                                   \
        float *xr = xo + node * KP;                                                             \
        if constexpr (AL16) *reinterpret_cast<v4f *>(xr) = v4f{acc01.x, acc01.y, acc23.x, acc23.y};   \
        else { xr[0] = acc01.x; xr[1] = acc01.y; xr[2] = acc23.x; xr[3] = acc23.y; }            \
        acc01 = v2f{0.f, 0.f}; acc23 = v2f{0.f, 0.f};                                           \
        ++node;                                                                                 \
        next_end = ipt[node + 1];                                                               \
    }
    int base = e_begin;
    for (; base + GB <= e_end; base += GB) {
        float w[GB];
        v4f x[GB];
        gather_batch<GB>(my_src, my_w, rsrc, voff0, w, x, std::make_integer_sequence<int, GB>{});
        const int nb = base + GB + gl;
        my_src = 0; my_w = 0.0f;
        if (nb < e_end) { my_src = gstream1(a.adj_src + nb); my_w = gstream1(a.adj_w + nb); }
#pragma unroll
        for (int u = 0; u < GB; ++u) {
            GNN_ROW_BOUNDARY(base + u)
            gather_fma(acc01, acc23, w[u], x[u]);
        }
    }
    {
        const int cnt = e_end - base;
        float w[GB];
        v4f x[GB];
        gather_batch<GB>(my_src, my_w, rsrc, voff0, w, x, std::make_integer_sequence<int, GB>{});
#pragma unroll
        for (int u = 0; u < GB; ++u) {
            if (u < cnt) {
                GNN_ROW_BOUNDARY(base + u)
                gather_fma(acc01, acc23, w[u], x[u]);
            }
        }
    }
#undef GNN_ROW_BOUNDARY
    for (; node < node_end; ++node) {
        float *xr = xo + node * KP;
        if constexpr (AL16) *reinterpret_cast<v4f *>(xr) = v4f{acc01.x, acc01.y, acc23.x, acc23.y};
        else { xr[0] = acc01.x; xr[1] = acc01.y; xr[2] = acc23.x; xr[3] = acc23.y; }
        acc01 = v2f{0.f, 0.f}; acc23 = v2f{0.f, 0.f};
    }
    own.write(a, X, i0, lane, KP, c_aggs);
}

template <bool AL16, int J>
__device__ __forceinline__ void prog_consume(int words, float w, v4f x, v2f &acc01, v2f &acc23, float *xo, int KP)
{
    gather_fma(acc01, acc23, w, x);
    const unsigned t = (unsigned)row_bcast_i<J>(words);
    if (t & GNN_GP_ROW_END) {
        float *xr = xo + __umul24(t & GNN_GP_ROW_MASK, (unsigned)KP);
        if constexpr (AL16) *reinterpret_cast<v4f *>(xr) = v4f{acc01.x, acc01.y, acc23.x, acc23.y};
        else { xr[0] = acc01.x; xr[1] = acc01.y; xr[2] = acc23.x; xr[3] = acc23.y; }
        acc01 = v2f{0.f, 0.f}; acc23 = v2f{0.f, 0.f};
    }
}
template <bool AL16, int GB, int... J>
__device__ __forceinline__ void prog_batch(int words, float my_w, __amdgpu_buffer_rsrc_t rsrc, int voff0, float (&w)[GB], v4f (&x)[GB],
                                           std::integer_sequence<int, J...>)
{
    ((w[J] = row_bcast_f<J>(my_w),
      x[J] = __builtin_bit_cast(v4f, __builtin_amdgcn_raw_buffer_load_b128(rsrc, (row_bcast_i<J>(words) & ~0xff) | voff0, 0, 0))), ...);
}
template <bool AL16, int GB, int... J>
__device__ __forceinline__ void prog_consume_all(int words, const float (&w)[GB], const v4f (&x)[GB], v2f &acc01, v2f &acc23, float *xo, int KP,
                                                 std::integer_sequence<int, J...>)
{
    (prog_consume<AL16, J>(words, w[J], x[J], acc01, acc23, xo, KP), ...);
}
typedef int v2i __attribute__((ext_vector_type(2)));
__device__ __forceinline__ v2i prog_header_request(const GnnFusedArgs &a, int tile)
{
    v2i h = {a.gp_last_first, tile == a.gp_tiles ? a.gp_last_nb : 0};
    if (tile < a.gp_tiles) h = *reinterpret_cast<const GNN_GLOBAL v2i *>(gptr(a.gp_hdr) + 2 * (int64_t)tile);
    return h;
}
__device__ __forceinline__ v2i prog_entry(const GnnFusedArgs &a, int b, int lane)
{
    return *reinterpret_cast<const GNN_GLOBAL v2i *>(gptr(a.gp_ent) + ((int64_t)b * 64 + lane) * 2);
}
template <bool AL16>
__device__ __forceinline__ void load_tile_prog64(const GnnFusedArgs &a, float *X, int64_t i0, int lane, int KP, int c_aggs, int first, int nb, v2i ent)
{
    constexpr int GB = 16;
    const int gl = lane & 15;
    TileOwn64<AL16> own;
    own.request(a, i0, lane);
    v2f acc01 = {0.f, 0.f}, acc23 = {0.f, 0.f};
    const __amdgpu_buffer_rsrc_t rsrc = __builtin_amdgcn_make_buffer_rsrc(const_cast<float *>(a.state_cur), 0, (int)a.state_bytes, 0x00020000);
    const int voff0 = gl * 16;
    float *xo = X + c_aggs + gl * 4;
    for (int b = 0; b < nb; ++b) {
        float w[GB];
        v4f x[GB];
        const int words = ent.x;
        prog_batch<AL16, GB>(words, __int_as_float(ent.y), rsrc, voff0, w, x, std::make_integer_sequence<int, GB>{});
        if (b + 1 < nb) ent = prog_entry(a, first + b + 1, lane);
        prog_consume_all<AL16, GB>(words, w, x, acc01, acc23, xo, KP, std::make_integer_sequence<int, GB>{});
    }
    own.write(a, X, i0, lane, KP, c_aggs);
}

#ifndef GNN_FIRST_BATCH_AHEAD
#define GNN_FIRST_BATCH_AHEAD 1
#endif
template <int GB, int... J>
__device__ __forceinline__ void prog_rows_request(int words, __amdgpu_buffer_rsrc_t rsrc, int voff0, v4f (&x)[GB], std::integer_sequence<int, J...>)
{
    ((x[J] = __builtin_bit_cast(v4f, __builtin_amdgcn_raw_buffer_load_b128(rsrc, (row_bcast_i<J>(words) & ~0xff) | voff0, 0, 0))), ...);
}
template <bool AL16, int GB, int... J>
__device__ __forceinline__ void prog_consume_first(v2i ent, const v4f (&x)[GB], v2f &acc01, v2f &acc23, float *xo, int KP, std::integer_sequence<int, J...>)
{
    (prog_consume<AL16, J>(ent.x, row_bcast_f<J>(__int_as_float(ent.y)), x[J], acc01, acc23, xo, KP), ...);
}
__device__ __forceinline__ void prog_first_batch_request(const GnnFusedArgs &a, int first, int nb, v2i ent0, int lane, v4f (&x0)[16], v2i &ent1)
{
    const __amdgpu_buffer_rsrc_t rsrc = __builtin_amdgcn_make_buffer_rsrc(const_cast<float *>(a.state_cur), 0, (int)a.state_bytes, 0x00020000);
    if (nb > 1) ent1 = prog_entry(a, first + 1, lane);
    __builtin_amdgcn_sched_barrier(0);
    prog_rows_request<16>(ent0.x, rsrc, (lane & 15) * 16, x0, std::make_integer_sequence<int, 16>{});
}
template <bool AL16>
__device__ __forceinline__ void load_tile_prog64_ahead(const GnnFusedArgs &a, float *X, int64_t i0, int lane, int KP, int c_aggs, int first, int nb,
                                                       v2i ent0, const v4f (&x0)[16], v2i ent, v2i hdr_next_raw, int &first_next, int &nb_next,
                                                       v2i &ent_next)
{
    constexpr int GB = 16;
    const int gl = lane & 15;
    TileOwn64<AL16> own;
    own.request(a, i0, lane);
    v2f acc01 = {0.f, 0.f}, acc23 = {0.f, 0.f};
    const __amdgpu_buffer_rsrc_t rsrc = __builtin_amdgcn_make_buffer_rsrc(const_cast<float *>(a.state_cur), 0, (int)a.state_bytes, 0x00020000);
    const int voff0 = gl * 16;
    float *xo = X + c_aggs + gl * 4;
    auto request_next = [&]() {
        first_next = __builtin_amdgcn_readfirstlane(hdr_next_raw.x); nb_next = __builtin_amdgcn_readfirstlane(hdr_next_raw.y);
        ent = v2i{(int)GNN_GP_NOROW, 0};
        if (nb_next > 0) ent = prog_entry(a, first_next, lane);
    };
    if (nb <= 1) request_next();
    prog_consume_first<AL16, GB>(ent0, x0, acc01, acc23, xo, KP, std::make_integer_sequence<int, GB>{});
    for (int b = 1; b < nb; ++b) {
        float w[GB];
        v4f x[GB];
        const int words = ent.x;
        prog_batch<AL16, GB>(words, __int_as_float(ent.y), rsrc, voff0, w, x, std::make_integer_sequence<int, GB>{});
        if (b + 1 < nb) ent = prog_entry(a, first + b + 1, lane);
        else request_next();
        prog_consume_all<AL16, GB>(words, w, x, acc01, acc23, xo, KP, std::make_integer_sequence<int, GB>{});
    }
    ent_next = ent;
    own.write(a, X, i0, lane, KP, c_aggs);
}

template <bool AL16>
__device__ __forceinline__ void load_tile_given64(const GnnFusedArgs &a, float *X, int64_t i0, int lane, int KP, int c_aggs)
{
    constexpr int Ds = 64;
    v4f own[8], agg[8];
    {
        const float *src = a.state_cur + (a.row_begin + i0) * Ds + lane * 4;
        const float *sag = a.agg_in + i0 * Ds + lane * 4;
#pragma unroll
        for (int u = 0; u < 8; ++u) {
            own[u] = gload4(src + u * 256);
            agg[u] = gload4(sag + u * 256);
        }
    }
    float lab[4];
    const int IW = a.IW, nlab = 32 * IW;
    {
        const float *src = a.inv + i0 * IW;
#pragma unroll
        for (int u = 0; u < 4; ++u) lab[u] = (lane + 64 * u < nlab) ? gload1(src + lane + 64 * u) : 0.0f;
    }
#pragma unroll
    for (int u = 0; u < 8; ++u) {
        float *x = X + (4 * u + (lane >> 4)) * KP + (lane & 15) * 4;
        if constexpr (AL16) { *reinterpret_cast<v4f *>(x) = own[u]; *reinterpret_cast<v4f *>(x + c_aggs) = agg[u]; }
        else {
            x[0] = own[u].x; x[1] = own[u].y; x[2] = own[u].z; x[3] = own[u].w;
            x[c_aggs] = agg[u].x; x[c_aggs + 1] = agg[u].y; x[c_aggs + 2] = agg[u].z; x[c_aggs + 3] = agg[u].w;
        }
    }
    const float inv_iw = 1.0f / (float)(IW > 0 ? IW : 1);
#pragma unroll
    for (int u = 0; u < 4; ++u) {
        const int t = lane + 64 * u;
        if (t < nlab) {
            const int i = (int)(((float)t + 0.5f) * inv_iw), c = t - i * IW;
            X[i * KP + label_col(c, Ds, a.NLc, c_aggs)] = lab[u];
        }
    }
    if (nlab > 256)
        for (int t = 256 + lane; t < nlab; t += 64) {
            const int i = t / IW, c = t - i * IW;
            X[i * KP + label_col(c, Ds, a.NLc, c_aggs)] = gload1(a.inv + i0 * IW + t);
        }
}

template <bool COH = false, bool STORE = true>
__device__ __forceinline__ void check_store_generic(const GnnFusedArgs &a, float *X, int64_t i0, int lane, int nvalid, int KP,
                                                 int c_aggs, int *moved_out = nullptr)
{
    const int Ds = a.Ds, half = lane >> 5;
    if constexpr (STORE) {
        float *dst = a.state_nxt + i0 * Ds;
        const int total = nvalid * Ds;
        RowCol rc(lane, Ds);
        for (int t = lane; t < total; t += 64, rc.next()) sstore1<COH>(dst + t, X[rc.i * KP + c_aggs + rc.c]);
    }
    const float *xo = X + (lane & 31) * KP, *xn = xo + c_aggs;
    float s_ = 0.0f;
    for (int f = 0; f < Ds; ++f) {
        const float o = xo[f];
        const float d = half ? o : (xn[f] - o);
        const float dd = d * d;
        s_ = s_ + dd;
    }
// ... 120 lines not shown
    float *xrow = X + (lane & 31) * KP;
    float d2 = 0.0f, o2 = 0.0f;
#pragma unroll
    for (int jt = 0; jt < 2; ++jt)
#pragma unroll
        for (int q = 0; q < 4; ++q) {
            const int f0 = 32 * jt + 8 * q + 4 * half;
            const v4f o = *reinterpret_cast<const v4f *>(xrow + f0);
            const v4f nw = {out[jt][4 * q], out[jt][4 * q + 1], out[jt][4 * q + 2], out[jt][4 * q + 3]};
            *reinterpret_cast<v4f *>(xrow + c_aggs + f0) = nw;
            const v4f d = nw - o;
            d2 = __builtin_fmaf(d.x, d.x, d2); d2 = __builtin_fmaf(d.y, d.y, d2); d2 = __builtin_fmaf(d.z, d.z, d2); d2 = __builtin_fmaf(d.w, d.w, d2);
            o2 = __builtin_fmaf(o.x, o.x, o2); o2 = __builtin_fmaf(o.y, o.y, o2); o2 = __builtin_fmaf(o.z, o.z, o2); o2 = __builtin_fmaf(o.w, o.w, o2);
        }
    d2 = d2 + shfl_f(d2, lane ^ 32);
    o2 = o2 + shfl_f(o2, lane ^ 32);
    const float root = sqrtf(d2), nrm = sqrtf(o2);
    {
        const bool voter = (lane & 31) < nvalid;
        const float rhs = a.thr * nrm, band = GNN_BAND_ABS * nrm + GNN_BAND_REL * rhs;
        const bool am = __any(voter && root > rhs), ar = __any(voter && root > rhs + band), ab = __any(voter && gnn_gate_borderline(root, rhs, band));
        if (lane == 0) gnn_flag_raise_certified(a.flag_out, am, ar, ab);
    }
    __builtin_amdgcn_fence(__ATOMIC_ACQ_REL, "wavefront");
    float *dst = a.state_nxt + i0 * 64 + lane * 4;
    const float *xs = X + (lane >> 4) * KP + c_aggs + (lane & 15) * 4;
    for (int u = 0; u < 8; ++u)
        if (4 * u + (lane >> 4) < nvalid) *reinterpret_cast<GNN_GLOBAL v4f *>(gptr_w(dst) + 256 * u) = *reinterpret_cast<const v4f *>(xs + 4 * u * KP);
}

__device__ __forceinline__ int tile_rowptr_request(const GnnFusedArgs &a, int tile, int lane)
{
    const int64_t i0 = (int64_t)tile * 32;
    if (i0 >= a.n_rows) return 0;
    const int nvalid = (int)((a.n_rows - i0) < 32 ? (a.n_rows - i0) : 32);
    return (lane <= nvalid) ? gstream1(a.indptr + i0 + lane) : 0;
}
__device__ __forceinline__ int tile_rowptr_clamp(const GnnFusedArgs &a, int tile, int lane, int raw)
{
    const int64_t i0 = (int64_t)tile * 32;
    if (i0 >= a.n_rows) return 0;
    const int nvalid = (int)((a.n_rows - i0) < 32 ? (a.n_rows - i0) : 32);
    const int last_ip = shfl_i(raw, nvalid);
    return lane <= nvalid ? raw : last_ip;
}
__device__ __forceinline__ void tile_first_ids(const GnnFusedArgs &a, int ip, int lane, int &src, float &w)
{
    const int gl = lane & 15, grp = lane >> 4;
    const int e_begin = shfl_i(ip, grp * 8), e_end = shfl_i(ip, grp * 8 + 8);
    src = 0; w = 0.0f;
    if (e_begin + gl < e_end) { src = gstream1(a.adj_src + e_begin + gl); w = gstream1(a.adj_w + e_begin + gl); }
}

template <int N>
__device__ __forceinline__ void zero_acc(f32x16 (&acc)[N])
{
#pragma unroll
    for (int jt = 0; jt < N; ++jt)
#pragma unroll
        for (int r = 0; r < 16; ++r) acc[jt][r] = 0.0f;
}

template <int LAYERS, int NT, int NTL, int ACT, bool SPLIT, bool FULL = false, bool GIVEN = false, int PC = 3, bool PROG = false, int ACTL = ACT>
__global__ void __launch_bounds__(GNN_FUSED_THREADS, 2) k_fused(const GnnFusedArgs a0)
{
    const GnnFusedArgs &a = a0;
    extern __shared__ __attribute__((aligned(16))) float lds[];
    if (!gnn_gate_open(a.gate, a.world)) return;
#ifdef GNN_DIAG
    if (a.lds_floats) {
        for (int t = threadIdx.x; t < a.lds_floats; t += blockDim.x) lds[t] = __builtin_nanf("");
        __syncthreads();
    }
#endif
    const int lane = threadIdx.x & 63, wave = __builtin_amdgcn_readfirstlane(threadIdx.x >> 6);
    const int KP = a.KP, Ds = a.Ds;
    float *X = lds + (size_t)wave * 32 * KP;
    const int c_aggs = a.c_aggs;
    const int W_launch = (int)gridDim.x * (int)(blockDim.x >> 6);
    const int w_launch = wave * (int)gridDim.x + (int)blockIdx.x;
    const bool third_round = (int64_t)2 * W_launch * 32 < a.n_rows;
    int tile = w_launch + a.tile_base, next_tile = w_launch + W_launch + a.tile_base;
    int ip_first_raw = 0;
    v2i hdr_first_raw = {0, 0};
    if constexpr (PROG) hdr_first_raw = prog_header_request(a, tile);
    else ip_first_raw = tile_rowptr_request(a, tile, lane);
    float *ep = lds + (size_t)GNN_FUSED_WAVES * 32 * KP + 32 + GNN_FUSED_WAVES * 36;
    for (int t = threadIdx.x; t < 3 * 32 * NTL; t += blockDim.x) {
        const int which = t / (32 * NTL), f = t - which * 32 * NTL;
        ep[t] = which == 0 ? a.bias[LAYERS - 1][f] * (SPLIT ? a.bsc[LAYERS - 1] : 1.0f) : (a.bn_scale ? (which == 1 ? a.bn_scale[f] : a.bn_shift[f]) : 0.0f);
    }
    float *hb = ep + 3 * 32 * NTL;
    if constexpr (SPLIT && LAYERS > 1)
        for (int t = threadIdx.x; t < (LAYERS - 1) * 32 * NT; t += blockDim.x)
            hb[t] = a.bias[t / (32 * NT)][t % (32 * NT)] * (ACT == GNN_ACT_SELU ? 1.44269504088896341f : 1.0f) * a.bsc[t / (32 * NT)];
    __syncthreads();
    if (a.stagger > 0) {
        int rounds = 0;
        if (a.variant & 4) rounds = wave >= GNN_FUSED_WAVES / 2 ? a.stagger : 0;
        else rounds = (int)((((unsigned)blockIdx.x * GNN_FUSED_WAVES + (unsigned)wave) * 0x9E3779B1u) >> 16) % (unsigned)(a.stagger + 1);
        for (int i = 0; i < rounds; ++i) __builtin_amdgcn_s_sleep(127);
    }
    int ip_cur = 0, src_cur = 0;
    float w_cur = 0.0f;
    constexpr bool AHEAD = PROG && GNN_FIRST_BATCH_AHEAD && !(SPLIT && PC == 3 && NT == 4);
    int hdr_first = 0, hdr_nb = 0;
    v2i ent_cur = {AHEAD ? (int)GNN_GP_NOROW : 0, 0}, ent_second = {0, 0};
    v4f x_first[16];
    if constexpr (PROG) {
        hdr_first = __builtin_amdgcn_readfirstlane(hdr_first_raw.x); hdr_nb = __builtin_amdgcn_readfirstlane(hdr_first_raw.y);
        if (hdr_nb > 0) ent_cur = prog_entry(a, hdr_first, lane);
        if constexpr (AHEAD) prog_first_batch_request(a, hdr_first, hdr_nb, ent_cur, lane, x_first, ent_second);
    } else {
        ip_cur = tile_rowptr_clamp(a, tile, lane, ip_first_raw);
        if (FULL || Ds == 64) tile_first_ids(a, ip_cur, lane, src_cur, w_cur);
    }
    if constexpr (FULL) zero_pad_columns(a, X, lane, KP);
  for (;;) {
    const int64_t i0 = (int64_t)tile * 32;
    if (i0 >= a.n_rows) break;
    const int nvalid = (int)((a0.n_rows - i0) < 32 ? (a0.n_rows - i0) : 32);
    GnnFusedArgs a = a0;
    asm volatile("" : "+s"(a.Wp[0]), "+s"(a.Wp[1]), "+s"(a.Wp[2]), "+s"(a.bias[0]), "+s"(a.bias[1]), "+s"(a.bias[2]));
    asm volatile("" : "+s"(a.bn_scale), "+s"(a.bn_shift), "+s"(a.state_cur), "+s"(a.state_nxt), "+s"(a.inv), "+s"(a.adj_src), "+s"(a.adj_w));
#ifndef GNN_DIAG
#define GNN_STAMP(slot) do { } while (0)
#else
    unsigned long long *stamp = a.stamps ? a.stamps + ((size_t)tile << 3) : nullptr;
#define GNN_STAMP(slot)                                                                      \
    do {                                                                                     \
        if (stamp) {                                                                         \
            __builtin_amdgcn_sched_barrier(0);                                               \
            const unsigned long long t_ = __builtin_amdgcn_s_memtime();                      \
            if (lane == 0) stamp[slot] = t_;                                                 \
            __builtin_amdgcn_sched_barrier(0);                                               \
        }                                                                                    \
    } while (0)
#endif
    GNN_STAMP(0);

    [[maybe_unused]] int *ipt = reinterpret_cast<int *>(lds + (size_t)GNN_FUSED_WAVES * 32 * KP + 32) + wave * 36;
    int ip_next_raw = 0;
    int hdr_first_next = 0, hdr_nb_next = 0;
    v2i ent_next = {0, 0};
    v2i hdr_next_raw = {0, 0};
    if constexpr (PROG) hdr_next_raw = prog_header_request(a, next_tile);
    else {
        if (lane <= 32) ipt[lane] = ip_cur;
        ip_next_raw = tile_rowptr_request(a, next_tile, lane);
    }
    const bool fast64 = FULL || ((Ds == 64) && (nvalid == 32) && !a.agg_in);
    if (a.variant & 1) __builtin_amdgcn_s_setprio(3);
    if constexpr (FULL && GIVEN) load_tile_given64<SPLIT>(a, X, i0, lane, KP, c_aggs);
    else if constexpr (AHEAD)
        load_tile_prog64_ahead<SPLIT>(a, X, i0, lane, KP, c_aggs, hdr_first, hdr_nb, ent_cur, x_first, ent_second, hdr_next_raw, hdr_first_next, hdr_nb_next, ent_next);
    else if constexpr (PROG) load_tile_prog64<SPLIT>(a, X, i0, lane, KP, c_aggs, hdr_first, hdr_nb, ent_cur);
    else if constexpr (FULL) load_tile_fast64<SPLIT, true>(a, X, ipt, i0, lane, KP, c_aggs, src_cur, w_cur);
    else {
        if (fast64) load_tile_fast64<SPLIT>(a, X, ipt, i0, lane, KP, c_aggs, src_cur, w_cur);
        else load_tile_generic(a, X, ipt, i0, lane, nvalid, KP, c_aggs);
    }
    if (a.variant & 1) __builtin_amdgcn_s_setprio(0);
    __builtin_amdgcn_fence(__ATOMIC_ACQ_REL, "wavefront");
    GNN_STAMP(2);

    const int half = lane >> 5;
    const float *xb = X + (lane & 31) * KP + half;
    f32x16 out[NTL];
    float mx = 0.0f;
    if constexpr (SPLIT) {
        const __amdgpu_buffer_rsrc_t wrs = __builtin_amdgcn_make_buffer_rsrc(const_cast<int *>(a.Ws_base), 0, a.ws_bytes, 0x00020000);
        const int wv = lane * 16;
        const float *xr = X + (lane & 31) * KP + 8 * half;
        if constexpr (LAYERS == 1) {
            layer0_split<NTL, false, PC>(xr, wrs, wv, a.ws_off[0], a.chunks0, out, ep, half, mx);
        } else {
            f32x16 h1[NT];
            if constexpr (FULL) layer0_split<NT, true, PC>(xr, wrs, wv, a.ws_off[0], a.chunks0, h1, hb, half, mx);
            else {
                if (Ds == 64) layer0_split<NT, true, PC>(xr, wrs, wv, a.ws_off[0], a.chunks0, h1, hb, half, mx);
                else layer0_split<NT, false, PC>(xr, wrs, wv, a.ws_off[0], a.chunks0, h1, hb, half, mx);
            }
            GNN_STAMP(3);
            GNN_STAMP(4);
            if constexpr (PC == 2) { asm volatile("" : "+v"(mx)); mx = __builtin_fmaxf(mx, hidden_range<NT>(h1, a.usc[0])); asm volatile("" : "+v"(mx)); }
            if constexpr (LAYERS == 2) {
                layer_split_from_regs<NT, NTL, ACT, PC>(h1, ep, half, out, wrs, wv, a.ws_off[1], a.usc[0], mx);
            } else {
                f32x16 h2[NT];
                layer_split_from_regs<NT, NT, ACT, PC>(h1, hb + 32 * NT, half, h2, wrs, wv, a.ws_off[1], a.usc[0], mx);
                if constexpr (PC == 2) { asm volatile("" : "+v"(mx)); mx = __builtin_fmaxf(mx, hidden_range<NT>(h2, a.usc[1])); asm volatile("" : "+v"(mx)); }
                layer_split_from_regs<NT, NTL, ACT, PC>(h2, ep, half, out, wrs, wv, a.ws_off[2], a.usc[1], mx);
            }
        }
    } else if constexpr (LAYERS == 1) {
        zero_acc<NTL>(out);
        layer_from_lds<NTL>(xb, a.Wp[0] + (size_t)lane * NTL, a.kk0, out, a.wstride);
    } else {
        f32x16 h1[NT];
        zero_acc<NT>(h1);
        layer_from_lds<NT>(xb, a.Wp[0] + (size_t)lane * NT, a.kk0, h1, a.wstride);
        GNN_STAMP(3);
        GNN_STAMP(4);
        if constexpr (LAYERS == 2) {
            zero_acc<NTL>(out);
            layer_from_regs<NT, NTL, ACT>(h1, a.bias[0], half, out, a.Wp[1] + (size_t)lane * NTL, a.wstride);
        } else {
            f32x16 h2[NT];
            zero_acc<NT>(h2);
            layer_from_regs<NT, NT, ACT>(h1, a.bias[0], half, h2, a.Wp[1] + (size_t)lane * NT, a.wstride);
            zero_acc<NTL>(out);
            layer_from_regs<NT, NTL, ACT>(h2, a.bias[1], half, out, a.Wp[2] + (size_t)lane * NTL, a.wstride);
        }
    }
    __builtin_amdgcn_fence(__ATOMIC_ACQ_REL, "wavefront");
    GNN_STAMP(5);
    if constexpr (AHEAD && SPLIT && PC == 2) gnn_flag_raise_range(a.flag_out, mx);
    int next2_tile = 0x3fffffff;
    if (third_round) {
        int64_t ctr_off = 0;
        if constexpr (AHEAD) asm volatile("" : "+v"(ctr_off));
        if constexpr (AHEAD) { if (lane == 0) next2_tile = atomicAdd(a0.tile_ctr + ctr_off, 1); }
        else if (lane == 0) next2_tile = atomicAdd(a0.tile_ctr, 1) + 2 * W_launch;
    }
    int ip_next = 0, src_next = 0;
    float w_next = 0.0f;
    if constexpr (AHEAD) { }
    else if constexpr (PROG) {
        hdr_first_next = __builtin_amdgcn_readfirstlane(hdr_next_raw.x); hdr_nb_next = __builtin_amdgcn_readfirstlane(hdr_next_raw.y);
        if (hdr_nb_next > 0) ent_next = prog_entry(a, hdr_first_next, lane);
    } else {
        ip_next = tile_rowptr_clamp(a, next_tile, lane, ip_next_raw);
        if (FULL || Ds == 64) tile_first_ids(a, ip_next, lane, src_next, w_next);
    }
    if constexpr (!AHEAD && SPLIT && PC == 2) gnn_flag_raise_range(a.flag_out, mx);
    GnnFlagPeek peek = {0, 0, 0};
    if (SPLIT && NTL == 2 && lane == 0) peek = gnn_flag_peek(a.flag_out);
    if constexpr (AHEAD) {
        __builtin_amdgcn_sched_barrier(0);
        prog_first_batch_request(a, hdr_first_next, hdr_nb_next, ent_next, lane, x_first, ent_second);
        __builtin_amdgcn_sched_barrier(0);
    }
    bool finished = false;
    if constexpr (SPLIT && NTL == 2) {
        if (fast64) {
#pragma unroll
            for (int jt = 0; jt < NTL; ++jt) {
                if (a.bn_scale) tile_epilogue_last<ACTL, true, true, true, true>(a.act_last, out[jt], ep, ep + 32 * NTL, ep + 64 * NTL, jt, half, 1 << 30, a.usc[LAYERS - 1]);
                else tile_epilogue_last<ACTL, false, true, true, true>(a.act_last, out[jt], ep, nullptr, nullptr, jt, half, 1 << 30, a.usc[LAYERS - 1]);
            }
            GNN_STAMP(6);
            if (nvalid == 32) finish_fast64_aligned<AHEAD>(a, X, out, i0, lane, KP, c_aggs, peek);
            else finish_fast64_partial(a, X, out, i0, lane, KP, c_aggs, nvalid);
            finished = true;
        }
    }
    if (!(FULL && SPLIT && NTL == 2) && !finished) {
#pragma unroll
        for (int jt = 0; jt < NTL; ++jt) {
            const float us = SPLIT ? a.usc[LAYERS - 1] : 1.0f;
            if (a.bn_scale) tile_epilogue_last<ACTL, true, SPLIT, true, SPLIT>(a.act_last, out[jt], ep, ep + 32 * NTL, ep + 64 * NTL, jt, half, 1 << 30, us);
            else tile_epilogue_last<ACTL, false, SPLIT, true, SPLIT>(a.act_last, out[jt], ep, nullptr, nullptr, jt, half, 1 << 30, us);
            float *x = X + (lane & 31) * KP + c_aggs;
#pragma unroll
            for (int r = 0; r < 16; ++r) {
                const int f = 32 * jt + (r & 3) + 8 * (r >> 2) + 4 * half;
                if (f < Ds) x[f] = out[jt][r];
            }
        }
        __builtin_amdgcn_fence(__ATOMIC_ACQ_REL, "wavefront");
        GNN_STAMP(6);
        if constexpr (FULL) {
            if (nvalid == 32) check_store_fast64(a, X, i0, lane, KP, c_aggs);
            else check_store_fast64_partial(a, X, i0, lane, KP, c_aggs, nvalid);
        } else {
            if (fast64) check_store_fast64(a, X, i0, lane, KP, c_aggs);
            else check_store_generic(a, X, i0, lane, nvalid, KP, c_aggs);
        }
    }
    GNN_STAMP(7);
#undef GNN_STAMP
    __builtin_amdgcn_fence(__ATOMIC_ACQ_REL, "wavefront");
    tile = next_tile;
    if constexpr (AHEAD) {
        asm volatile("" : "+v"(next2_tile));
        next_tile = __builtin_amdgcn_readfirstlane(next2_tile) + (third_round ? 2 * W_launch : 0) + a0.tile_base;
    } else next_tile = __builtin_amdgcn_readfirstlane(next2_tile) + a0.tile_base;
    ip_cur = ip_next; src_cur = src_next; w_cur = w_next;
    hdr_first = hdr_first_next; hdr_nb = hdr_nb_next; ent_cur = ent_next;
  }
}

template <int LAYERS, int NT, int NTL, int ACT, bool SPLIT, int ACTL, bool FULL, bool GIVEN = false, int PC = 3, bool PROG = false>
inline void launch_one_pc(const GnnFusedArgs &a, unsigned grid, size_t lds_bytes, hipStream_t st)
{
    if constexpr (FULL && !GIVEN && !PROG) {
        if (a.gp_tiles > 0) { launch_one_pc<LAYERS, NT, NTL, ACT, SPLIT, ACTL, FULL, GIVEN, PC, true>(a, grid, lds_bytes, st); return; }
    }
    static bool lds_raised[64] = {false};
    (void)gnn_raise_dynamic_lds(reinterpret_cast<const void *>(&k_fused<LAYERS, NT, NTL, ACT, SPLIT, FULL, GIVEN, PC, PROG, ACTL>), 160 * 1024, lds_raised);
    hipLaunchKernelGGL((k_fused<LAYERS, NT, NTL, ACT, SPLIT, FULL, GIVEN, PC, PROG, ACTL>), grid, a.threads ? a.threads : GNN_FUSED_THREADS, lds_bytes, st, a);
}
template <int LAYERS, int NT, int NTL, int ACT, bool SPLIT, int ACTL, bool FULL, bool GIVEN = false>
inline void launch_one(const GnnFusedArgs &a, unsigned grid, size_t lds_bytes, hipStream_t st)
{
    if (SPLIT && a.pieces == 2) launch_one_pc<LAYERS, NT, NTL, ACT, SPLIT, ACTL, FULL, GIVEN, 2>(a, grid, lds_bytes, st);
    else launch_one_pc<LAYERS, NT, NTL, ACT, SPLIT, ACTL, FULL, GIVEN, 3>(a, grid, lds_bytes, st);
}

template <int LAYERS, int NT, int NTL, int ACT, bool SPLIT, int ACTL>
inline void launch(const GnnFusedArgs &a, unsigned grid, size_t lds_bytes, hipStream_t st)
{
    if constexpr (NTL == 2) {
        if (a.full_tiles && a.agg_in) { launch_one<LAYERS, NT, NTL, ACT, SPLIT, ACTL, true, true>(a, grid, lds_bytes, st); return; }
        if (a.full_tiles) { launch_one<LAYERS, NT, NTL, ACT, SPLIT, ACTL, true>(a, grid, lds_bytes, st); return; }
    }
    launch_one<LAYERS, NT, NTL, ACT, SPLIT, ACTL, false>(a, grid, lds_bytes, st);
}

template <int LAYERS, int ACT, bool SPLIT, int ACTL = ACT>
inline bool launch_tiles(int nt, int ntl, const GnnFusedArgs &a, unsigned grid, size_t lds_bytes, hipStream_t st)
{
    if constexpr (LAYERS == 1) {
        if (ntl == 1) launch<1, 1, 1, ACT, SPLIT, ACTL>(a, grid, lds_bytes, st);
        else if (ntl == 2) launch<1, 2, 2, ACT, SPLIT, ACTL>(a, grid, lds_bytes, st);
        else if (ntl == 4) launch<1, 4, 4, ACT, SPLIT, ACTL>(a, grid, lds_bytes, st);
        else return false;
    } else {
        if (nt == 1 && ntl == 1) launch<LAYERS, 1, 1, ACT, SPLIT, ACTL>(a, grid, lds_bytes, st);
        else if (nt == 2 && ntl == 2) launch<LAYERS, 2, 2, ACT, SPLIT, ACTL>(a, grid, lds_bytes, st);
        else if (nt == 4 && ntl == 2) launch<LAYERS, 4, 2, ACT, SPLIT, ACTL>(a, grid, lds_bytes, st);
        else if (nt == 4 && ntl == 4) launch<LAYERS, 4, 4, ACT, SPLIT, ACTL>(a, grid, lds_bytes, st);
        else return false;
    }
    return true;
}

template <class F>
inline bool dispatch_act(int act, F &&f)
{
    switch (act) {
    case GNN_ACT_LINEAR: return f(std::integral_constant<int, GNN_ACT_LINEAR>{});
    case GNN_ACT_RELU: return f(std::integral_constant<int, GNN_ACT_RELU>{});
    case GNN_ACT_SELU: return f(std::integral_constant<int, GNN_ACT_SELU>{});
    case GNN_ACT_ELU: return f(std::integral_constant<int, GNN_ACT_ELU>{});
    case GNN_ACT_TANH: return f(std::integral_constant<int, GNN_ACT_TANH>{});
    case GNN_ACT_SIGMOID: return f(std::integral_constant<int, GNN_ACT_SIGMOID>{});
    default: return false;
    }
}

template <int LAYERS, bool SPLIT>
inline bool launch_act(int act, int nt, int ntl, const GnnFusedArgs &a, unsigned grid, size_t lds_bytes, hipStream_t st)
{
    return dispatch_act(act, [&](auto A) { return launch_tiles<LAYERS, A.value, SPLIT>(nt, ntl, a, grid, lds_bytes, st); });
}

template <int LAYERS, bool SPLIT>
inline bool launch_act_mixed(int act, int nt, int ntl, const GnnFusedArgs &a, unsigned grid, size_t lds_bytes, hipStream_t st)
{
    static_assert(LAYERS >= 2, "a one-layer net has one activation");
    return dispatch_act(act, [&](auto A) { return launch_tiles<LAYERS, A.value, SPLIT, GNN_ACTL_FROM_ARGS>(nt, ntl, a, grid, lds_bytes, st); });
}

}
```

### gnn_tf_2.x_amd/csrc/gnn_graph.hip

```cpp
#include <stdlib.h>
#include <string.h>

#include "gnn_engine.h"

static hipStream_t g_fill_stream[64] = {nullptr};

static int fill_stream(int device, hipStream_t *st)
{
    if (device < 0 || device >= 64) return gnn_fail(GNN_ERR_ARG, "device %d out of range", device);
    if (!g_fill_stream[device]) HIPCHK(hipStreamCreateWithFlags(&g_fill_stream[device], hipStreamNonBlocking));
    *st = g_fill_stream[device];
    return GNN_OK;
}

static int graph_zero_fill(gnn_graph *g, void *p, size_t bytes)
{
    hipStream_t st = nullptr;
    int rc = fill_stream(g->device, &st);
    if (rc) return rc;
#ifdef GNN_DIAG
    static const bool legacy = getenv("GNN_LEGACY_NULL_MEMSET") != nullptr;
    if (legacy) { HIPCHK(hipMemset(p, 0, bytes)); return GNN_OK; }
#endif
    if (!g->ready) HIPCHK(hipEventCreateWithFlags(&g->ready, hipEventDisableTiming));
    if ((rc = zero_on_stream(p, bytes, st))) return rc;
    HIPCHK(hipEventRecord(g->ready, st));
    return GNN_OK;
}

int gnn_graph_wait_ready(const gnn_graph *g, hipStream_t st)
{
    if (g && g->ready) HIPCHK(hipStreamWaitEvent(st, g->ready, 0));
    return GNN_OK;
}

__global__ void k_relabel(int64_t N, int NLb, const float *__restrict__ base_nodes, int Ds, GnnStateTabs tabs,
                          const int *kfinal, int get_state, int T, const float *__restrict__ out,
                          const uint8_t *__restrict__ mask, const int32_t *__restrict__ mask_pos, int get_output,
                          float *__restrict__ dst, int NLd)
{
    const int64_t t = (int64_t)blockIdx.x * blockDim.x + threadIdx.x;
    if (t >= N * NLd) return;
    const int64_t i = t / NLd;
    int c = (int)(t - i * NLd);
    float v;
    if (c < NLb) {
        v = base_nodes[i * NLb + c];
    } else {
        c -= NLb;
        if (get_state && c < Ds) {
            const float *state = gnn_state_after(tabs, *kfinal);
            v = state[i * Ds + c];
        } else {
            if (get_state) c -= Ds;
            v = mask[i] ? out[(int64_t)mask_pos[i] * T + c] : 0.0f;
        }
    }
    dst[t] = v;
}

__global__ void k_arc_base(int64_t E, int ALb, const float *__restrict__ base, int ALd, float *__restrict__ dst)
{
    const int64_t t = (int64_t)blockIdx.x * blockDim.x + threadIdx.x;
    if (t >= E * ALd) return;
    const int64_t p = t / ALd;
    const int c = (int)(t - p * ALd);
    dst[t] = c < ALb ? base[p * ALb + c] : 0.0f;
}

__global__ void k_arc_scatter(int64_t M, int T, const int32_t *__restrict__ rows, const float *__restrict__ out, int ALb, int ALd, float *__restrict__ dst)
{
    const int64_t t = (int64_t)blockIdx.x * blockDim.x + threadIdx.x;
    if (t >= M * T) return;
    const int64_t m = t / T;
    const int c = (int)(t - m * T);
    dst[(int64_t)rows[m] * ALd + ALb + c] = out[t];
}

__global__ void k_arc_permute(int64_t E, int AL, const int32_t *__restrict__ arc_id, const float *__restrict__ orig, float *__restrict__ csr)
{
    const int64_t t = (int64_t)blockIdx.x * blockDim.x + threadIdx.x;
    if (t >= E * AL) return;
    const int64_t q = t / AL;
    const int c = (int)(t - q * AL);
    csr[t] = orig[(int64_t)arc_id[q] * AL + c];
}

static void graph_release_shared(gnn_graph_shared *sh)
{
    if (!sh || --sh->refs > 0) return;
    (void)hipFree(sh->indptr); (void)hipFree(sh->adj_src); (void)hipFree(sh->masked_rows);
    (void)hipFree(sh->adj_w); (void)hipFree(sh->arc_w); (void)hipFree(sh->arc_labels); (void)hipFree(sh->mask);
    (void)hipFree(sh->src_indptr); (void)hipFree(sh->src_dst); (void)hipFree(sh->src_w);
    (void)hipFree(sh->arc_id); (void)hipFree(sh->arc_labels_orig);
    (void)hipFree(sh->full_indptr); (void)hipFree(sh->full_src); (void)hipFree(sh->full_w);
    (void)hipFree(sh->gp_hdr); (void)hipFree(sh->gp_ent);
    delete sh;
}

static int graph_create_impl(int64_t n_index, int64_t n_global, int64_t row_begin, int64_t own_off, int64_t n_rows, int64_t n_arcs,
                             const int32_t *indptr, const int32_t *adj_src, const float *adj_w, const float *arc_w,
                             const float *arc_labels, int dim_arc_label, const float *nodes, int dim_node_label,
                             const uint8_t *mask, int device, gnn_graph **out)
{
    ARGCHK(out, "out is NULL");
    *out = nullptr;
    ARGCHK(n_index > 0 && n_index < (int64_t)1 << 31 && n_global > 0 && n_global < (int64_t)1 << 31, "n_nodes=%lld out of range", (long long)n_global);
    ARGCHK(row_begin >= 0 && n_rows >= 0 && row_begin + n_rows <= n_global && own_off >= 0 && own_off + n_rows <= n_index,
           "owned rows [%lld,+%lld) outside [0,%lld)", (long long)row_begin, (long long)n_rows, (long long)n_global);
    ARGCHK(n_arcs >= 0 && n_arcs < (int64_t)1 << 31, "n_arcs=%lld out of range", (long long)n_arcs);
    ARGCHK(dim_node_label > 0 && dim_arc_label >= 0, "label dims must be NL>0, AL>=0");
    ARGCHK(indptr && nodes && mask, "indptr/nodes/mask are required");
    ARGCHK(n_arcs == 0 || (adj_src && adj_w && arc_w && (arc_labels || dim_arc_label == 0)), "arc arrays are required");
    ARGCHK(indptr[0] == 0 && indptr[n_rows] == n_arcs, "indptr[0]=%d, indptr[n_rows]=%d, n_arcs=%lld", indptr[0],
           indptr[n_rows], (long long)n_arcs);
    int maxdeg = 0;
    for (int64_t r = 0; r < n_rows; ++r) {
        const int d = indptr[r + 1] - indptr[r];
        ARGCHK(d >= 0, "indptr not monotone at row %lld", (long long)r);
        maxdeg = std::max(maxdeg, d);
    }
    for (int64_t e = 0; e < n_arcs; ++e)
        ARGCHK(adj_src[e] >= 0 && adj_src[e] < n_index, "adj_src[%lld]=%d outside [0,%lld)", (long long)e, adj_src[e], (long long)n_index);

    HIPCHK(hipSetDevice(device));
    gnn_graph *g = new gnn_graph();
    g->device = device; g->N = n_index; g->N_global = n_global; g->row_begin = row_begin; g->own_off = own_off; g->n_rows = n_rows; g->E = n_arcs;
    g->NL = dim_node_label; g->AL = dim_arc_label; g->base_NL = dim_node_label; g->base_AL = dim_arc_label;
    g->nodes_rows = n_index;
    g->sh = new gnn_graph_shared();
    g->sh->max_degree = maxdeg;
    std::vector<int32_t> rows, pos((size_t)n_rows);
    for (int64_t r = 0; r < n_rows; ++r) { pos[r] = (int32_t)rows.size(); if (mask[r]) rows.push_back((int32_t)r); }
    g->n_masked = (int64_t)rows.size();
    std::vector<int32_t> both(rows);
    both.insert(both.end(), pos.begin(), pos.end());
    int rc = 0;
    if ((rc = dev_upload(&g->sh->indptr, indptr, (size_t)n_rows + 1)) || (rc = dev_upload(&g->sh->adj_src, adj_src, (size_t)n_arcs)) ||
        (rc = dev_upload(&g->sh->adj_w, adj_w, (size_t)n_arcs)) || (rc = dev_upload(&g->sh->arc_w, arc_w, (size_t)n_arcs)) ||
        (rc = dev_upload(&g->sh->arc_labels, arc_labels, (size_t)n_arcs * dim_arc_label)) ||
        (rc = dev_upload(&g->sh->mask, mask, (size_t)n_rows)) || (rc = dev_upload(&g->sh->masked_rows, both.data(), both.size())) ||
        (rc = dev_upload(&g->nodes, nodes, (size_t)n_index * dim_node_label))) {
        gnn_graph_destroy(g);
        return rc;
    }
    *out = g;
    return GNN_OK;
}

extern "C" int gnn_graph_create(int64_t n_nodes, int64_t row_begin, int64_t n_rows, int64_t n_arcs,
                                const int32_t *indptr, const int32_t *adj_src, const float *adj_w, const float *arc_w,
                                const float *arc_labels, int dim_arc_label, const float *nodes, int dim_node_label,
                                const uint8_t *mask, int device, gnn_graph **out)
{
    return graph_create_impl(n_nodes, n_nodes, row_begin, row_begin, n_rows, n_arcs, indptr, adj_src, adj_w, arc_w, arc_labels, dim_arc_label,
                             nodes, dim_node_label, mask, device, out);
}

extern "C" int gnn_graph_create_halo(int64_t n_nodes_global, int rank, int world, int64_t halo_block, int64_t n_send, const int32_t *send_rows,
                                     int64_t n_arcs, const int32_t *indptr, const int32_t *adj_src_replica, const float *adj_w,
                                     const float *arc_w, const float *arc_labels, int dim_arc_label, const float *nodes_replica,
                                     int dim_node_label, const uint8_t *mask, int device, gnn_graph **out)
{
    ARGCHK(out, "out is NULL");
    *out = nullptr;
    ARGCHK(world >= 2 && rank >= 0 && rank < world && halo_block >= 0 && n_send >= 0 && n_send <= halo_block && (n_send == 0 || send_rows), "bad halo description");
    int64_t rb = 0, nr = 0;
    int rc = gnn_shard_range(n_nodes_global, rank, world, &rb, &nr);
    if (rc) return rc;
    const int64_t shard = ((n_nodes_global + world - 1) / world + 31) / 32 * 32;
    for (int64_t j = 0; j < n_send; ++j)
        ARGCHK(send_rows[j] >= 0 && send_rows[j] < nr && (j == 0 || send_rows[j] > send_rows[j - 1]), "send_rows must be ascending owned-row indices");
    const int64_t n_index = shard + (int64_t)world * halo_block;
    rc = graph_create_impl(n_index, n_nodes_global, rb, 0, nr, n_arcs, indptr, adj_src_replica, adj_w, arc_w, arc_labels, dim_arc_label, nodes_replica,
                           dim_node_label, mask, device, out);
    if (rc) return rc;
    gnn_graph *g = *out;
    g->halo_world = world; g->halo_rank = rank; g->halo_block = halo_block; g->halo_count = n_send;
    rc = dev_upload(&g->halo_send, send_rows, (size_t)n_send);
// ... 247 lines not shown
```

### gnn_tf_2.x_amd/csrc/gnn_loop.hip

```cpp
#include <stdio.h>
#include <stdlib.h>
#include <string.h>

#include "gnn_engine.h"

__global__ void k_finalize(const int *flags, int world, int max_iter, int *kfinal)
{
    const int lane = threadIdx.x;
    int k_final = max_iter;
    for (int k0 = 0; k0 < max_iter; k0 += 64) {
        const int k = k0 + lane;
        const bool closed = k < max_iter && !gnn_gate_open(flags + (size_t)k * world * GNN_FLAG_WORDS, world);
        const unsigned long long m = __ballot(closed);
        if (m) { k_final = k0 + __builtin_ctzll(m); break; }
    }
    if (lane == 0) { kfinal[0] = k_final; kfinal[1] = 0; }
    int amb = 0;
    const int last = k_final < max_iter ? k_final : max_iter - 1;
    for (int k = 1 + lane; k <= last; k += 64) {
        const int *gate = flags + (size_t)k * world * GNN_FLAG_WORDS;
        int robust = 0, border = 0;
#pragma unroll 16
        for (int p = 0; p < world * GNN_FLAG_SLOTS; ++p) { robust |= gate[p * GNN_FLAG_STRIDE + 1]; border |= gate[p * GNN_FLAG_STRIDE + 2]; }
        amb |= (!robust && border) ? 1 : 0;
// ... 254 lines not shown
    if (!rc && hipEventCreate(&l->ev_total[1]) != hipSuccess) rc = gnn_fail(GNN_ERR_HIP, "hipEventCreate");
    if (rc) { gnn_loop_destroy(l); return rc; }
    l->impl_req = 2;
    (void)maxw_s;
    if (comm && comm->grp) comm->grp->member[rank] = l;
    *out = l;
    return GNN_OK;
}

static int loop_ensure_unfused(gnn_loop *l)
{
    if (l->inp) return GNN_OK;
    int maxw = 1;
    for (int i = 1; i <= l->st->n_layers; ++i) maxw = std::max(maxw, l->st->dims[i]);
    int rc = dev_alloc(&l->inp, (size_t)l->g->n_rows * l->in_s);
    for (int b = 0; b < 2 && !rc; ++b) rc = dev_alloc(&l->tmp[b], (size_t)l->g->n_rows * maxw);
    return rc;
}

extern "C" int gnn_loop_set_impl(gnn_loop *l, int impl, int *used)
{
    ARGCHK(l && impl >= 0 && impl <= 2, "impl must be 0 (unfused), 1 (fused, exact f32 MFMA) or 2 (fused, split bf16 MFMA)");
    l->impl_req = impl;
    const int rc = gnn_loop_decide_form(l);
    if (used) *used = gnn_loop_impl_used(l);
    return rc;
}

extern "C" int gnn_loop_set_pieces(gnn_loop *l, int pieces, int *used)
{
    ARGCHK(l && (pieces == 2 || pieces == 3), "pieces must be 2 (fp16 x 2) or 3 (bf16 x 3)");
    l->pieces = pieces;
    if (used) *used = pieces;
    return GNN_OK;
}

extern "C" int gnn_loop_range_info(const gnn_loop *l, int *last_run_repeated, int *repeats_total)
{
    ARGCHK(l, "loop is NULL");
    if (last_run_repeated) *last_run_repeated = l->last_run_range_rerun ? 1 : 0;
    if (repeats_total) *repeats_total = l->range_reruns;
    return GNN_OK;
}

extern "C" int gnn_loop_gate_info(const gnn_loop *l, int *last_run_repeated, int *repeats_total)
{
    ARGCHK(l, "loop is NULL");
    if (last_run_repeated) *last_run_repeated = l->last_run_rerun ? 1 : 0;
    if (repeats_total) *repeats_total = l->certified_reruns;
    return GNN_OK;
}

extern "C" int gnn_loop_drop_cached_aggregates(gnn_loop *l)
{
    ARGCHK(l, "loop is NULL");
    l->inv_version = 0;
    return GNN_OK;
}

extern "C" int gnn_loop_set_persistent(gnn_loop *l, int enable, int *used)
{
    ARGCHK(l, "loop is NULL");
    l->small_disabled = enable == 0;
    const int rc = gnn_loop_decide_form(l);
    if (used) *used = l->form.path == GNN_PATH_PERSISTENT ? 1 : 0;
    return rc;
}

extern "C" int gnn_loop_set_tile_form(gnn_loop *l, int form, int *used)
{
    ARGCHK(l && form >= 0 && form <= 2, "form must be 0 (library's choice), 1 (one wave per tile) or 2 (wave pair per tile)");
    l->tile_form = form;
    const int rc = gnn_loop_decide_form(l);
    if (used) *used = l->form.path == GNN_PATH_UNFUSED ? 0 : (l->form.kernel == GNN_BODY_PAIR ? 2 : 1);
    return rc;
}

extern "C" int gnn_loop_set_gather_form(gnn_loop *l, int form, int *used)
{
    ARGCHK(l && form >= 0 && form <= 2, "form must be 0 (library's choice), 1 (walk the CSR) or 2 (the graph's gather program)");
    l->gather_form = form;
    const int rc = gnn_loop_decide_form(l);
    if (used) *used = l->form.path == GNN_PATH_UNFUSED ? 0 : (l->form.program ? 2 : 1);
    return rc;
}

extern "C" int gnn_loop_set_profiling(gnn_loop *l, int enable)
{
    ARGCHK(l, "loop is NULL");
    l->profiling = enable != 0;
    return GNN_OK;
}

extern "C" int gnn_loop_get_timing(const gnn_loop *l, float *total_ms, float *avg_iter_ms, int *n_iter_timed)
{
    ARGCHK(l, "loop is NULL");
    if (!l->ran) return gnn_fail(GNN_ERR_STATE, "gnn_loop_run has not been called");
    if (total_ms) *total_ms = l->total_ms;
    if (avg_iter_ms) *avg_iter_ms = l->avg_iter_ms;
    if (n_iter_timed) *n_iter_timed = l->n_iter_timed;
    return GNN_OK;
}

extern "C" int gnn_loop_get_exchange_timing(const gnn_loop *l, float *avg_between_bodies_ms)
{
    ARGCHK(l && avg_between_bodies_ms, "bad arguments");
    if (!l->ran) return gnn_fail(GNN_ERR_STATE, "gnn_loop_run has not been called");
    *avg_between_bodies_ms = l->avg_gap_ms;
    return GNN_OK;
}

extern "C" int gnn_counters_get(const gnn_loop *l, double *bytes_per_iteration, double *flops_per_iteration, int *iterations, float *total_ms,
                                float *avg_iteration_ms)
{
    ARGCHK(l, "loop is NULL");
    const gnn_graph *g = l->g;
    const double n = (double)g->n_rows, e = (double)g->E, ds = (double)l->Ds;
    if (bytes_per_iteration) *bytes_per_iteration = e * (4.0 * ds + 8.0) + 4.0 * (n + 1.0) + n * (8.0 * ds + 4.0 * (2.0 * l->NLc + g->AL));
    if (flops_per_iteration) {
        double f = 0.0;
        for (int i = 0; i < l->st->n_layers; ++i) f += 2.0 * (double)l->st->dims[i] * (double)l->st->dims[i + 1];
        *flops_per_iteration = n * f + 2.0 * e * ds;
    }
    if (iterations) *iterations = l->ran ? l->kfinal : 0;
    if (total_ms) *total_ms = l->ran ? l->total_ms : 0.f;
    if (avg_iteration_ms) *avg_iteration_ms = l->ran ? l->avg_iter_ms : 0.f;
    return GNN_OK;
}

extern "C" int gnn_loop_set_state0(gnn_loop *l, const float *state0, uint64_t seed)
{
    ARGCHK(l, "loop is NULL");
    HIPCHK(hipSetDevice(l->device));
    const gnn_graph *g = l->g;
    const size_t cnt = (size_t)g->n_rows * l->Ds;
    if (!l->state_init && l->D) {
        const size_t rows = l->world == 1 ? (size_t)std::max<int64_t>(l->N_pad, g->n_rows) : (size_t)g->n_rows;
        int rc = dev_alloc(&l->state_init, rows * l->Ds);
        if (!rc && rows > (size_t)g->n_rows) rc = zero_on_stream(l->state_init + cnt, sizeof(float) * (rows - (size_t)g->n_rows) * l->Ds, l->stream);
        if (rc) return rc;
    }
    float *own = l->state_init;
    if (l->D == 0) {
        l->have_state0 = true;
        return GNN_OK;
    }
    if (state0) {
        HIPCHK(hipMemcpyAsync(own, state0, cnt * sizeof(float), hipMemcpyHostToDevice, l->stream));
        HIPCHK(hipStreamSynchronize(l->stream));
    } else if (cnt) {
        hipLaunchKernelGGL(k_randn, cdiv((int64_t)cnt, 256), 256, 0, l->stream, (int64_t)cnt, (int64_t)g->row_begin * l->Ds, seed, 0.1f, own);
        HIPCHK(hipGetLastError());
        HIPCHK(hipStreamSynchronize(l->stream));
    }
    l->have_state0 = true;
    return GNN_OK;
}

extern "C" int gnn_loop_set_slice_exchange(gnn_loop *l, int on)
{
    ARGCHK(l, "loop is NULL");
    if (!on) { l->slice_mode = false; return GNN_OK; }
    ARGCHK(l->world > 1, "the feature-sliced exchange needs a communicator");
    ARGCHK(l->Ds % l->world == 0, "state width %d is not a multiple of the world size %d", l->Ds, l->world);
    ARGCHK(l->g->sh->full_indptr, "call gnn_graph_set_full_adjacency first (on this graph or on the graph it was derived from)");
    ARGCHK(!l->g->halo_world, "not on a boundary-exchange shard");
// ... 585 lines not shown
```

### include/gnn_hip.h

```cpp
#ifndef GNN_HIP_H
#define GNN_HIP_H

#include <stdint.h>

#ifdef __cplusplus
extern "C" {
#endif

typedef enum {
    GNN_OK = 0,
    GNN_ERR_ARG = -1,
    GNN_ERR_HIP = -2,
    GNN_ERR_STATE = -3,
    GNN_ERR_COMM = -4,
    GNN_ERR_UNSUPPORTED = -5
} gnn_status;

typedef enum {
    GNN_ACT_LINEAR = 0, GNN_ACT_RELU = 1, GNN_ACT_SELU = 2, GNN_ACT_ELU = 3,
    GNN_ACT_TANH = 4, GNN_ACT_SIGMOID = 5, GNN_ACT_SOFTMAX = 6
} gnn_activation;

typedef struct gnn_graph gnn_graph;
typedef struct gnn_mlp gnn_mlp;
typedef struct gnn_loop gnn_loop;
typedef struct gnn_comm gnn_comm;

const char *gnn_last_error(void);
int gnn_version(void);
int gnn_device_count(int *count);
int gnn_device_synchronize(int device);

int gnn_graph_create(int64_t n_nodes, int64_t row_begin, int64_t n_rows, int64_t n_arcs, const int32_t *indptr,
                     const int32_t *adj_src, const float *adj_w, const float *arc_w, const float *arc_labels,
                     int dim_arc_label, const float *nodes, int dim_node_label, const uint8_t *mask, int device,
                     gnn_graph **out);
int gnn_graph_create_from_arcs(int64_t n_nodes, int64_t n_arcs, const int32_t *arc_src, const int32_t *arc_dst,
                               const float *arc_labels, int dim_arc_label, int aggregation_mode, const float *nodes,
                               int dim_node_label, const uint8_t *mask, int device, gnn_graph **out,
                               int32_t *indptr_out, int32_t *adj_src_out, float *adj_w_out, int32_t *arc_id_out,
                               float *arc_w_out);
int gnn_graph_derive(const gnn_graph *base, int extra_node_label_dims, gnn_graph **out);
int gnn_graph_update_labels(gnn_graph *dst, const gnn_graph *base, const gnn_loop *from, int get_state, int get_output);
int gnn_graph_set_arc_order(gnn_graph *g, const int32_t *arc_id, const float *arc_labels_orig);
int gnn_graph_derive_edge(const gnn_graph *base, int extra_nodes, int extra_arcs, gnn_graph **out);
int gnn_graph_get_nodes(const gnn_graph *g, float *nodes_out );
int gnn_graph_dims(const gnn_graph *g, int64_t *n_nodes, int64_t *n_rows, int64_t *n_arcs, int *dim_node_label,
                   int *dim_arc_label, int64_t *n_masked);
int gnn_graph_destroy(gnn_graph *g);

int gnn_mlp_create(int n_layers, const int32_t *dims, const int32_t *acts, const float *const *W, const float *const *b,
                   const float *bn, float bn_eps, int device, gnn_mlp **out);
int gnn_mlp_set_weights(gnn_mlp *m, const float *const *W, const float *const *b, const float *bn);
int gnn_mlp_forward(gnn_mlp *m, int64_t n_rows, const float *x, float *y);
int gnn_mlp_get_weights(gnn_mlp *m, float *const *W, float *const *b, float *bn);
int gnn_mlp_reset_optimizer(gnn_mlp *m);
int gnn_mlp_destroy(gnn_mlp *m);

int gnn_loop_create(gnn_graph *g, gnn_mlp *net_state, gnn_mlp *net_output, int state_dim, int max_iter, float threshold,
                    gnn_comm *comm , gnn_loop **out);
int gnn_loop_set_state0(gnn_loop *l, const float *state0, uint64_t seed);
int gnn_loop_run(gnn_loop *l, int training, float *k_out);
int gnn_loop_run_many(gnn_loop **loops, int n, float *k_out);
int gnn_loop_get_state(const gnn_loop *l, float *state_out );
int gnn_loop_get_output(const gnn_loop *l, float *out , int64_t *n_masked);
int gnn_loop_readout(const gnn_loop *l, int n_graphs, const int32_t *ng_indptr, const int32_t *ng_node,
                     const float *ng_w, float *out_graph );
int gnn_loop_set_edge_readout(gnn_loop *l, const int32_t *entry_dst, const float *arc_labels, const uint8_t *arc_mask);
int gnn_loop_train_step(gnn_loop *l, const int32_t *src_indptr, const int32_t *src_dst, const float *src_w,
                        const float *targets, const float *sample_weights, int64_t n_targets, int loss_kind,
                        int n_graphs, const int32_t *ng_indptr, const int32_t *ng_node, const float *ng_w,
                        const float *dropout_state, const float *dropout_output, const uint8_t *masks_state,
                        const uint8_t *masks_output, uint64_t seed, const float *bn_state, const float *bn_output,
                        float *loss_out, float *k_out, float *grads_state, float *grads_output,
                        float *bn_batch_state, float *bn_batch_output);
int gnn_loop_train_forward(gnn_loop *l, const int32_t *src_indptr, const int32_t *src_dst, const float *src_w,
                           const float *dropout_state, const float *dropout_output, const uint8_t *masks_state,
                           const uint8_t *masks_output, uint64_t seed, const float *bn_state, const float *bn_output,
                           float *k_out, float *out_nodes);
int gnn_loop_train_backward(gnn_loop *l, const float *d_out_nodes, const float *d_state_extra, float *grads_state,
                            float *grads_output, float *bn_batch_state, float *bn_batch_output, float *d_nodes,
                            float *d_arc_labels);
int gnn_loop_update_moving_statistics(gnn_loop *l, float bn_momentum_state, float bn_momentum_output);
int gnn_loop_arm_optimizer(gnn_loop *l, int kind, const float *hyper, int mean, float bn_momentum_state, float bn_momentum_output);
int gnn_loop_optimizer_step(gnn_loop *l, int kind, const float *hyper, float state_grad_scale, float bn_momentum_state,
                            float bn_momentum_output);
int gnn_loss_grad(int loss_kind, int64_t n_rows, int n_out, const float *targets, const float *out,
                  const float *sample_weights, double *loss, float *d_out);
int gnn_loss_grad_ex(int loss_kind, int64_t n_rows, int n_out, const float *targets, const float *out,
                     const float *sample_weights, double label_smoothing, double huber_delta, double *loss, float *d_out);
int gnn_loop_set_loss_params(gnn_loop *l, double label_smoothing, double huber_delta);
int gnn_mlp_set_regularizers(gnn_mlp *m, const double *l1, const double *l2);
int gnn_loop_set_clipping(gnn_loop *l, double clipvalue, double clipnorm, double global_clipnorm);
int gnn_loop_grad_sqnorm(gnn_loop *l, float state_grad_scale, double *sqnorm, double *penalty);
int gnn_loop_optimizer_step_scaled(gnn_loop *l, int kind, const float *hyper, float state_grad_scale, double grad_scale,
                                   float bn_momentum_state, float bn_momentum_output);
int gnn_loop_set_impl(gnn_loop *l, int impl, int *used);
int gnn_loop_gate_info(const gnn_loop *l, int *last_run_repeated, int *repeats_total);
int gnn_loop_set_pieces(gnn_loop *l, int pieces, int *used);
int gnn_loop_range_info(const gnn_loop *l, int *last_run_repeated, int *repeats_total);
int gnn_split_f16_exponent(float max_abs);
void gnn_split_f16(const float *v, int n, int e, uint16_t *p0, uint16_t *p1);
int gnn_loop_set_persistent(gnn_loop *l, int enable, int *used);
int gnn_loop_set_tile_form(gnn_loop *l, int form, int *used);
int gnn_loop_set_gather_form(gnn_loop *l, int form, int *used);
int gnn_gather_program_build(int64_t n_rows, const int32_t *indptr, const int32_t *adj_src, const float *adj_w, int32_t *hdr, int32_t *ent,
                             int64_t *n_batches);
int gnn_graph_gather_program_info(const gnn_graph *g, int64_t *tiles, int64_t *batches, int64_t *bytes, float *build_ms);
enum { GNN_FORM_PER_OP = 0, GNN_FORM_MLP_FWD = 1, GNN_FORM_WIDE = 2, GNN_FORM_CHAIN3 = 3, GNN_FORM_WGRAD_BF = 4, GNN_FORM_WGRAD_F32 = 5 };
int gnn_train_forms(int n_layers, const int *dims, const int *acts, const float *rates, int64_t n_rows, int producer_dropout, int *out);
int gnn_loop_train_forms(const gnn_loop *l, int net, int *out);
#define GNN_TRAIN_PERSISTENT_MAX_BYTES (256u << 20)
int gnn_loop_set_train_persistent(gnn_loop *l, int enable, int *used);
int gnn_train_persistent_form(int n_layers, const int *dims, const int *acts, const float *rates, int64_t n_rows, int max_iter, int *out);
int gnn_loop_train_info(const gnn_loop *l, int *out);
int gnn_loop_train_mask(const gnn_loop *l, int net, int body, int pos, uint8_t *out, int64_t *count);
int gnn_fused_net_form(int n_layers, const int *dims, const int *acts, int n_label_cols_in_concat, int *out);
int gnn_small_form(int n_layers, const int *dims, const int *acts, int n_label_cols_in_concat, int64_t n_rows, int *out);
int gnn_loop_set_profiling(gnn_loop *l, int enable);
int gnn_loop_drop_cached_aggregates(gnn_loop *l);
int gnn_loop_get_timing(const gnn_loop *l, float *total_ms, float *avg_iter_ms, int *n_iter_timed);
int gnn_loop_get_exchange_timing(const gnn_loop *l, float *avg_between_bodies_ms);
int gnn_counters_get(const gnn_loop *l, double *bytes_per_iteration, double *flops_per_iteration, int *iterations, float *total_ms,
                     float *avg_iteration_ms);
int gnn_lgnn_run(gnn_loop *const *loops, gnn_graph *const *graphs, int n_layers, int get_state, int get_output, float *k_out);
int gnn_loop_destroy(gnn_loop *l);

int gnn_shard_range(int64_t n_nodes, int rank, int world, int64_t *row_begin, int64_t *n_rows);
int gnn_comm_unique_id(uint8_t id[128]);
int gnn_comm_create(const uint8_t id[128], int rank, int world, int device, gnn_comm **out);
int gnn_comm_allreduce_max(gnn_comm *c, double *value);
int gnn_comm_destroy(gnn_comm *c);
int gnn_halo_plan(int64_t n_nodes, int world, const int32_t *indptr, const int32_t *adj_src, int32_t *slot ,
                  int64_t *counts , int64_t *block);
int gnn_graph_create_halo(int64_t n_nodes_global, int rank, int world, int64_t halo_block, int64_t n_send, const int32_t *send_rows,
                          int64_t n_arcs, const int32_t *indptr, const int32_t *adj_src_replica, const float *adj_w,
                          const float *arc_w, const float *arc_labels, int dim_arc_label, const float *nodes_replica,
                          int dim_node_label, const uint8_t *mask, int device, gnn_graph **out);
int gnn_graph_set_full_adjacency(gnn_graph *g, int64_t n_global, const int32_t *indptr, const int32_t *adj_src, const float *adj_w);
int gnn_loop_set_slice_exchange(gnn_loop *l, int on);
int gnn_comm_create_loopback(int world, int device, gnn_comm **out );
int gnn_loop_run_group(gnn_loop **loops, int n, float *k_out);
int gnn_loop_readout_group(gnn_loop **loops, int n, int n_graphs, const int32_t *ng_indptr, const int32_t *ng_node,
                           const float *ng_w, float *out_graph);
int gnn_graph_update_labels_group(gnn_graph **dsts, gnn_graph *const *bases, gnn_loop *const *froms, int n, int get_state,
                                  int get_output);

#ifdef __cplusplus
}
#endif
#endif
```

Before: 1.813 billion node-state-updates/s.

## Add cost-balanced tile schedule for the gather-program fused kernel

```diff
diff --git a/gnn_tf_2.x_amd/GNN/_engine.py b/gnn_tf_2.x_amd/GNN/_engine.py
--- a/gnn_tf_2.x_amd/GNN/_engine.py
+++ b/gnn_tf_2.x_amd/GNN/_engine.py
@@ -18,7 +18,7 @@
            'gnn_loss_grad_ex', 'gnn_loop_set_loss_params', 'gnn_train_forms', 'gnn_loop_train_forms', 'gnn_loop_train_mask', 'gnn_fused_net_form', 'gnn_small_form',
            'gnn_loop_set_train_persistent', 'gnn_train_persistent_form', 'gnn_loop_train_info',
            'gnn_mlp_set_regularizers', 'gnn_loop_set_clipping', 'gnn_loop_grad_sqnorm', 'gnn_loop_optimizer_step_scaled',
-           'gnn_counters_get', 'gnn_lgnn_run', 'gnn_loop_run_many', 'gnn_loop_set_impl', 'gnn_loop_gate_info', 'gnn_loop_set_pieces', 'gnn_loop_range_info', 'gnn_split_f16_exponent', 'gnn_split_f16', 'gnn_loop_set_persistent', 'gnn_loop_set_tile_form', 'gnn_loop_set_gather_form', 'gnn_gather_program_build', 'gnn_graph_gather_program_info', 'gnn_loop_drop_cached_aggregates', 'gnn_loop_set_profiling', 'gnn_loop_get_timing', 'gnn_loop_get_exchange_timing', 'gnn_loop_destroy', 'gnn_shard_range',
+           'gnn_counters_get', 'gnn_lgnn_run', 'gnn_loop_run_many', 'gnn_loop_set_impl', 'gnn_loop_gate_info', 'gnn_loop_set_pieces', 'gnn_loop_range_info', 'gnn_split_f16_exponent', 'gnn_split_f16', 'gnn_loop_set_persistent', 'gnn_loop_set_tile_form', 'gnn_loop_set_gather_form', 'gnn_gather_program_build', 'gnn_graph_gather_program_info', 'gnn_loop_set_tile_schedule', 'gnn_tile_schedule_build', 'gnn_graph_tile_schedule_info', 'gnn_loop_drop_cached_aggregates', 'gnn_loop_set_profiling', 'gnn_loop_get_timing', 'gnn_loop_get_exchange_timing', 'gnn_loop_destroy', 'gnn_shard_range',
            'gnn_comm_unique_id', 'gnn_comm_create', 'gnn_comm_allreduce_max', 'gnn_comm_destroy', 'gnn_halo_plan', 'gnn_graph_create_halo',
            'gnn_comm_create_loopback', 'gnn_graph_set_full_adjacency', 'gnn_loop_set_slice_exchange', 'gnn_loop_run_group', 'gnn_loop_readout_group', 'gnn_graph_update_labels_group']
 
@@ -174,6 +174,14 @@
     ent = np.zeros((nb.value, 64, 2), np.int32)
     _check(lib().gnn_gather_program_build(C.c_int64(n_rows), _ip(indptr), _ip(adj_src), _fp(adj_w), None, _ip(ent), C.byref(nb)))
     return hdr, ent.view(np.uint32)
+
+
+def tile_schedule(cost, waves: int, kind: int):
+    cost = np.ascontiguousarray(cost, dtype=np.int64)
+    order = np.full(cost.size, -1, np.int32)
+    _check(lib().gnn_tile_schedule_build(C.c_int64(cost.size), cost.ctypes.data_as(C.POINTER(C.c_int64)), C.c_int64(int(waves)), C.c_int(int(kind)),
+                                         _ip(order)))
+    return order
 
 
 def halo_plan(n_nodes: int, world: int, indptr, adj_src):
@@ -301,6 +309,11 @@
         t, b, n, ms = C.c_int64(0), C.c_int64(0), C.c_int64(0), C.c_float(0)
         _check(lib().gnn_graph_gather_program_info(self._h, C.byref(t), C.byref(b), C.byref(n), C.byref(ms)))
         return dict(tiles=t.value, batches=b.value, bytes=n.value, build_ms=ms.value)
+
+    def tile_schedule_info(self) -> dict:
+        s, k, b, t, ms = C.c_int64(0), C.c_int(0), C.c_int64(0), C.c_int64(0), C.c_float(0)
+        _check(lib().gnn_graph_tile_schedule_info(self._h, C.byref(s), C.byref(k), C.byref(b), C.byref(t), C.byref(ms)))
+        return dict(slots=s.value, kind=k.value, body=b.value, tail=t.value, build_ms=ms.value)
 
     def set_arc_order(self, arc_id, arc_labels_orig) -> None:
         arc_id = np.ascontiguousarray(arc_id, dtype=np.int32)
@@ -702,6 +715,11 @@
         _check(lib().gnn_loop_set_gather_form(self._h, C.c_int(int(form)), C.byref(used)))
         return used.value
 
+    def set_tile_schedule(self, kind: int) -> int:
+        used = C.c_int(0)
+        _check(lib().gnn_loop_set_tile_schedule(self._h, C.c_int(int(kind)), C.byref(used)))
+        return used.value
+
     def counters(self) -> dict:
         b, f, it, tot, avg = C.c_double(), C.c_double(), C.c_int(), C.c_float(), C.c_float()
         _check(lib().gnn_counters_get(self._h, C.byref(b), C.byref(f), C.byref(it), C.byref(tot), C.byref(avg)))
diff --git a/gnn_tf_2.x_amd/csrc/gnn_build.hip b/gnn_tf_2.x_amd/csrc/gnn_build.hip
--- a/gnn_tf_2.x_amd/csrc/gnn_build.hip
+++ b/gnn_tf_2.x_amd/csrc/gnn_build.hip
@@ -258,6 +258,81 @@
     return GNN_OK;
 }
 
+extern "C" int gnn_tile_schedule_build(int64_t slots, const int64_t *cost, int64_t waves, int kind, int32_t *order)
+{
+    ARGCHK(slots >= 0 && slots < (int64_t)1 << 31 && order && (cost || kind == 0 || slots == 0), "slots / cost / order are required");
+    ARGCHK(waves > 0 && (kind == 0 || kind == 1), "waves must be positive, kind 0 (identity) or 1 (balanced)");
+    if (kind == 0) {
+        for (int64_t s = 0; s < slots; ++s) order[s] = (int32_t)s;
+        return GNN_OK;
+    }
+    try {
+        std::vector<int32_t> sorted((size_t)slots);
+        for (int64_t s = 0; s < slots; ++s) sorted[s] = (int32_t)s;
+        std::sort(sorted.begin(), sorted.end(), [&](int32_t x, int32_t y) { return cost[x] != cost[y] ? cost[x] > cost[y] : x < y; });
+        const int64_t K = std::min(2 * waves, slots / 2), M = slots - K;
+        const int64_t S = GNN_TILE_SCHEDULE_STRATA, C = (M + S - 1) / S;
+        int64_t p = 0;
+        for (int64_t q = 0; q < C; ++q)
+            for (int64_t r = 0; r < S; ++r)
+                if (r * C + q < M) order[p++] = sorted[r * C + q];
+        for (int64_t t = M; t < slots; ++t) order[p++] = sorted[t];
+    } catch (const std::bad_alloc &) { return gnn_fail(GNN_ERR_HIP, "no host memory for a schedule of %lld tiles", (long long)slots); }
+    return GNN_OK;
+}
+
+bool gnn_tile_schedule_ensure(const gnn_graph *g, int kind, int64_t waves)
+{
+    gnn_graph_shared *sh = g->sh;
+    if (!sh->gp_ent || kind < 0 || kind > 1) return false;
+    if (sh->gp_slot[kind]) return kind == 0 || sh->gp_sched_waves == waves;
+    if (kind == 1 && sh->gp_sched_tried) return false;
+    if (kind == 1) sh->gp_sched_tried = true;
+    const int64_t slots = (int64_t)sh->gp_cost.size();
+    int dev_before = -1;
+    if (hipGetDevice(&dev_before) != hipSuccess || hipSetDevice(g->device) != hipSuccess) { (void)hipGetLastError(); return false; }
+    const auto t0 = std::chrono::steady_clock::now();
+    int32_t *d_slot = nullptr;
+    bool ok = false;
+    try {
+        std::vector<int32_t> order((size_t)slots), slot((size_t)slots * 4);
+        ok = gnn_tile_schedule_build(slots, sh->gp_cost.data(), waves, kind, order.data()) == GNN_OK;
+        for (int64_t s = 0; ok && s < slots; ++s) {
+            const int32_t t = order[s];
+            slot[4 * s] = sh->gp_hdr_host[2 * (size_t)t]; slot[4 * s + 1] = sh->gp_hdr_host[2 * (size_t)t + 1]; slot[4 * s + 2] = t; slot[4 * s + 3] = 0;
+        }
+        ok = ok && gnn_dev_malloc((void **)&d_slot, sizeof(int32_t) * std::max<size_t>(4, slot.size())) == hipSuccess &&
+             hipMemcpy(d_slot, slot.data(), sizeof(int32_t) * slot.size(), hipMemcpyHostToDevice) == hipSuccess;
+    } catch (const std::bad_alloc &) { ok = false; }
+    if (ok) {
+        sh->gp_slot[kind] = d_slot;
+        if (kind == 1) {
+            sh->gp_sched_waves = waves;
+            sh->gp_sched_tail = std::min(2 * waves, slots / 2);
+            sh->gp_sched_ms = std::chrono::duration<float, std::milli>(std::chrono::steady_clock::now() - t0).count();
+        }
+    } else {
+        (void)hipFree(d_slot);
+        (void)hipGetLastError();
+    }
+    (void)hipSetDevice(dev_before);
+    return ok;
+}
+
+extern "C" int gnn_graph_tile_schedule_info(const gnn_graph *g, int64_t *slots, int *kind, int64_t *body, int64_t *tail, float *build_ms)
+{
+    ARGCHK(g, "graph is NULL");
+    const gnn_graph_shared *sh = g->sh;
+    const bool have = sh->gp_ent != nullptr, balanced = have && sh->gp_slot[1] != nullptr;
+    const int64_t n = have ? (int64_t)sh->gp_cost.size() : 0;
+    if (slots) *slots = n;
+    if (kind) *kind = balanced ? 2 : (have ? 1 : 0);
+    if (body) *body = balanced ? n - sh->gp_sched_tail : n;
+    if (tail) *tail = balanced ? sh->gp_sched_tail : 0;
+    if (build_ms) *build_ms = balanced ? sh->gp_sched_ms : 0.0f;
+    return GNN_OK;
+}
+
 int gnn_gather_program_ensure(const gnn_graph *g)
 {
     gnn_graph_shared *sh = g->sh;
@@ -271,6 +346,8 @@
     int32_t *d_hdr = nullptr, *d_ent = nullptr;
     int64_t batches = 0, last_batches = 0;
     int32_t last_hdr[2] = {0, 0};
+    std::vector<int32_t> hdr_host;
+    std::vector<int64_t> cost;
     bool ok = false;
     try {
         std::vector<int32_t> indptr((size_t)g->n_rows + 1), hdr((size_t)tiles * 2), src, ent;
@@ -295,10 +372,22 @@
              gnn_dev_malloc((void **)&d_ent, sizeof(int32_t) * ent.size()) == hipSuccess &&
              hipMemcpy(d_hdr, hdr.data(), sizeof(int32_t) * hdr.size(), hipMemcpyHostToDevice) == hipSuccess &&
              hipMemcpy(d_ent, ent.data(), sizeof(int32_t) * ent.size(), hipMemcpyHostToDevice) == hipSuccess;
+        if (ok) {
+            hdr_host = hdr;
+            if (rem) { hdr_host.push_back((int32_t)batches); hdr_host.push_back(last_hdr[1]); }
+            cost.resize((size_t)(tiles + (rem ? 1 : 0)));
+            for (size_t t = 0; t < cost.size(); ++t) cost[t] = (int64_t)indptr[(t + 1) * 32] - indptr[t * 32];
+        }
     } catch (const std::bad_alloc &) { ok = false; }
     if (ok) {
         sh->gp_hdr = d_hdr; sh->gp_ent = d_ent; sh->gp_tiles = tiles; sh->gp_batches = batches + last_batches;
         sh->gp_rows = g->n_rows; sh->gp_last_first = (int32_t)batches; sh->gp_last_nb = (int32_t)last_batches;
+        sh->gp_hdr_host.swap(hdr_host); sh->gp_cost.swap(cost);
+        if (!gnn_tile_schedule_ensure(g, 0, 1)) {
+            (void)hipFree(d_hdr); (void)hipFree(d_ent);
+            sh->gp_hdr = sh->gp_ent = nullptr; sh->gp_tiles = sh->gp_batches = 0;
+            (void)hipGetLastError();
+        }
         sh->gp_build_ms = std::chrono::duration<float, std::milli>(std::chrono::steady_clock::now() - t0).count();
     } else {
         (void)hipFree(d_hdr); (void)hipFree(d_ent);
diff --git a/gnn_tf_2.x_amd/csrc/gnn_common.h b/gnn_tf_2.x_amd/csrc/gnn_common.h
--- a/gnn_tf_2.x_amd/csrc/gnn_common.h
+++ b/gnn_tf_2.x_amd/csrc/gnn_common.h
@@ -159,6 +159,12 @@
     int32_t gp_last_first = 0, gp_last_nb = 0;
     bool gp_tried = false;
     float gp_build_ms = 0.0f;
+    int32_t *gp_slot[2] = {nullptr, nullptr};
+    std::vector<int32_t> gp_hdr_host;
+    std::vector<int64_t> gp_cost;
+    int64_t gp_sched_waves = 0, gp_sched_tail = 0;
+    bool gp_sched_tried = false;
+    float gp_sched_ms = 0.0f;
 };
 
 struct gnn_graph {
@@ -272,6 +278,7 @@
     int impl_req = 1;
     int tile_form = 0;
     int gather_form = 0;
+    int tile_schedule = 0;
     LoopForm form;
     int32_t *ng_ip = nullptr, *ng_node = nullptr;
     float *ng_w = nullptr, *ng_out = nullptr, *ng_part = nullptr;
@@ -327,6 +334,8 @@
 int gnn_loop_decide_form(gnn_loop *l);
 inline int gnn_loop_impl_used(const gnn_loop *l) { return l->form.path == GNN_PATH_UNFUSED ? 0 : (l->form.split ? 2 : 1); }
 int gnn_gather_program_ensure(const gnn_graph *g);
+constexpr int GNN_TILE_SCHEDULE_STRATA = 61;
+bool gnn_tile_schedule_ensure(const gnn_graph *g, int kind, int64_t waves);
 int gnn_fused_prepare(gnn_loop *l);
 int gnn_fused_pack(gnn_mlp *m, int nlc);
 int gnn_fused_iteration(gnn_loop *l, int k);
diff --git a/gnn_tf_2.x_amd/csrc/gnn_fused.h b/gnn_tf_2.x_amd/csrc/gnn_fused.h
--- a/gnn_tf_2.x_amd/csrc/gnn_fused.h
+++ b/gnn_tf_2.x_amd/csrc/gnn_fused.h
@@ -42,8 +42,8 @@
     int full_tiles;
     int variant;
     const float *agg_in;
-    const int32_t *gp_hdr, *gp_ent;
-    int gp_tiles, gp_last_first, gp_last_nb;
+    const int32_t *gp_hdr, *gp_ent, *gp_slot;
+    int gp_tiles, gp_last_first, gp_last_nb, gp_slots;
     int threads;
     int single_ticket;
     unsigned long long *stamps;
@@ -98,6 +98,7 @@
     bool split = false;
     int pieces = 3;
     bool program = false;
+    int schedule = 0;
     FusedPlan plan;
     unsigned grid = 0;
     size_t lds = 0;
diff --git a/gnn_tf_2.x_amd/csrc/gnn_fused.hip b/gnn_tf_2.x_amd/csrc/gnn_fused.hip
--- a/gnn_tf_2.x_amd/csrc/gnn_fused.hip
+++ b/gnn_tf_2.x_amd/csrc/gnn_fused.hip
@@ -16,10 +16,15 @@
 constexpr int K_SLACK = 8;
 
 constexpr int GNN_FUSED_VARIANT_DEFAULT = 1;
-constexpr int GNN_FUSED_SPREAD_DEFAULT = 8;
+#ifndef GNN_FUSED_SPREAD_DEFAULT
+#define GNN_FUSED_SPREAD_DEFAULT 8
+#endif
 constexpr int GNN_FUSED_SPREAD_SMALL_DEFAULT = 6;
 #ifndef GNN_GATHER_FORM_DEFAULT
 #define GNN_GATHER_FORM_DEFAULT 2
+#endif
+#ifndef GNN_TILE_SCHEDULE_DEFAULT
+#define GNN_TILE_SCHEDULE_DEFAULT 2
 #endif
 constexpr int S_SLACK = 2;
 
@@ -429,6 +434,7 @@
         if (f.program) {
             a.gp_hdr = g->sh->gp_hdr; a.gp_ent = g->sh->gp_ent; a.gp_tiles = (int)g->sh->gp_tiles;
             a.gp_last_first = g->sh->gp_last_first; a.gp_last_nb = g->sh->gp_last_nb;
+            a.gp_slot = g->sh->gp_slot[f.schedule == 2 ? 1 : 0]; a.gp_slots = (int)g->sh->gp_cost.size();
         }
     }
     a.lds_floats = gnn_poison_enabled() ? (int)(f.lds / sizeof(float)) : 0;
@@ -530,6 +536,11 @@
     if (f.kernel == GNN_BODY_FULL_TILE && !l->slice_mode && (l->gather_form ? l->gather_form : GNN_GATHER_FORM_DEFAULT) == 2 &&
         gnn_gather_program_ensure(g) == GNN_OK)
         f.program = g->sh->gp_ent != nullptr && g->sh->gp_rows == g->n_rows;
+    if (f.program) {
+        const int64_t waves = (int64_t)GNN_FUSED_WAVES * n_cu;
+        const int want = l->tile_schedule ? l->tile_schedule : (n_tiles >= 4 * waves ? GNN_TILE_SCHEDULE_DEFAULT : 1);
+        f.schedule = want == 2 && gnn_tile_schedule_ensure(g, 1, waves) ? 2 : 1;
+    }
     const SmallForm sf = small_form(l->st, p, g->n_rows);
     const bool persistent = l->world == 1 && !l->small_disabled && !l->profiling && sf.tile != 0;
     f.path = persistent ? GNN_PATH_PERSISTENT : GNN_PATH_BODIES;
diff --git a/gnn_tf_2.x_amd/csrc/gnn_fused_kernel.h b/gnn_tf_2.x_amd/csrc/gnn_fused_kernel.h
--- a/gnn_tf_2.x_amd/csrc/gnn_fused_kernel.h
+++ b/gnn_tf_2.x_amd/csrc/gnn_fused_kernel.h
@@ -917,10 +917,10 @@
     (prog_consume<AL16, J>(words, w[J], x[J], acc01, acc23, xo, KP), ...);
 }
 typedef int v2i __attribute__((ext_vector_type(2)));
-__device__ __forceinline__ v2i prog_header_request(const GnnFusedArgs &a, int tile)
-{
-    v2i h = {a.gp_last_first, tile == a.gp_tiles ? a.gp_last_nb : 0};
-    if (tile < a.gp_tiles) h = *reinterpret_cast<const GNN_GLOBAL v2i *>(gptr(a.gp_hdr) + 2 * (int64_t)tile);
+__device__ __forceinline__ v4i prog_header_request(const GnnFusedArgs &a, int slot)
+{
+    v4i h = {0, 0, a.gp_slots, 0};
+    if (slot < a.gp_slots) h = *reinterpret_cast<const GNN_GLOBAL v4i *>(gptr(a.gp_slot) + 4 * (int64_t)slot);
     return h;
 }
 __device__ __forceinline__ v2i prog_entry(const GnnFusedArgs &a, int b, int lane)
@@ -971,8 +971,8 @@
 }
 template <bool AL16>
 __device__ __forceinline__ void load_tile_prog64_ahead(const GnnFusedArgs &a, float *X, int64_t i0, int lane, int KP, int c_aggs, int first, int nb,
-                                                       v2i ent0, const v4f (&x0)[16], v2i ent, v2i hdr_next_raw, int &first_next, int &nb_next,
-                                                       v2i &ent_next)
+                                                       v2i ent0, const v4f (&x0)[16], v2i ent, v4i hdr_next_raw, int &first_next, int &nb_next,
+                                                       int &tid_next, v2i &ent_next)
 {
     constexpr int GB = 16;
     const int gl = lane & 15;
@@ -984,6 +984,7 @@
     float *xo = X + c_aggs + gl * 4;
     auto request_next = [&]() {
         first_next = __builtin_amdgcn_readfirstlane(hdr_next_raw.x); nb_next = __builtin_amdgcn_readfirstlane(hdr_next_raw.y);
+        tid_next = __builtin_amdgcn_readfirstlane(hdr_next_raw.z);
         ent = v2i{(int)GNN_GP_NOROW, 0};
         if (nb_next > 0) ent = prog_entry(a, first_next, lane);
     };
@@ -1270,7 +1271,7 @@
     const bool third_round = (int64_t)2 * W_launch * 32 < a.n_rows;
     int tile = w_launch + a.tile_base, next_tile = w_launch + W_launch + a.tile_base;
     int ip_first_raw = 0;
-    v2i hdr_first_raw = {0, 0};
+    v4i hdr_first_raw = {0, 0, 0, 0};
     if constexpr (PROG) hdr_first_raw = prog_header_request(a, tile);
     else ip_first_raw = tile_rowptr_request(a, tile, lane);
     float *ep = lds + (size_t)GNN_FUSED_WAVES * 32 * KP + 32 + GNN_FUSED_WAVES * 36;
@@ -1292,11 +1293,12 @@
     int ip_cur = 0, src_cur = 0;
     float w_cur = 0.0f;
     constexpr bool AHEAD = PROG && GNN_FIRST_BATCH_AHEAD && !(SPLIT && PC == 3 && NT == 4);
-    int hdr_first = 0, hdr_nb = 0;
+    int hdr_first = 0, hdr_nb = 0, tid = 0;
     v2i ent_cur = {AHEAD ? (int)GNN_GP_NOROW : 0, 0}, ent_second = {0, 0};
     v4f x_first[16];
     if constexpr (PROG) {
         hdr_first = __builtin_amdgcn_readfirstlane(hdr_first_raw.x); hdr_nb = __builtin_amdgcn_readfirstlane(hdr_first_raw.y);
+        tid = __builtin_amdgcn_readfirstlane(hdr_first_raw.z);
         if (hdr_nb > 0) ent_cur = prog_entry(a, hdr_first, lane);
         if constexpr (AHEAD) prog_first_batch_request(a, hdr_first, hdr_nb, ent_cur, lane, x_first, ent_second);
     } else {
@@ -1305,8 +1307,8 @@
     }
     if constexpr (FULL) zero_pad_columns(a, X, lane, KP);
   for (;;) {
-    const int64_t i0 = (int64_t)tile * 32;
-    if (i0 >= a.n_rows) break;
+    const int64_t i0 = (int64_t)(PROG ? tid : tile) * 32;
+    if (PROG ? tile >= a.gp_slots : i0 >= a.n_rows) break;
     const int nvalid = (int)((a0.n_rows - i0) < 32 ? (a0.n_rows - i0) : 32);
     GnnFusedArgs a = a0;
     asm volatile("" : "+s"(a.Wp[0]), "+s"(a.Wp[1]), "+s"(a.Wp[2]), "+s"(a.bias[0]), "+s"(a.bias[1]), "+s"(a.bias[2]));
@@ -1314,7 +1316,7 @@
 #ifndef GNN_DIAG
 #define GNN_STAMP(slot) do { } while (0)
 #else
-    unsigned long long *stamp = a.stamps ? a.stamps + ((size_t)tile << 3) : nullptr;
+    unsigned long long *stamp = a.stamps ? a.stamps + ((size_t)(PROG ? tid : tile) << 3) : nullptr;
 #define GNN_STAMP(slot)                                                                      \
     do {                                                                                     \
         if (stamp) {                                                                         \
@@ -1329,9 +1331,9 @@
 
     [[maybe_unused]] int *ipt = reinterpret_cast<int *>(lds + (size_t)GNN_FUSED_WAVES * 32 * KP + 32) + wave * 36;
     int ip_next_raw = 0;
-    int hdr_first_next = 0, hdr_nb_next = 0;
+    int hdr_first_next = 0, hdr_nb_next = 0, tid_next = 0;
     v2i ent_next = {0, 0};
-    v2i hdr_next_raw = {0, 0};
+    v4i hdr_next_raw = {0, 0, 0, 0};
     if constexpr (PROG) hdr_next_raw = prog_header_request(a, next_tile);
     else {
         if (lane <= 32) ipt[lane] = ip_cur;
@@ -1341,8 +1343,12 @@
     if (a.variant & 1) __builtin_amdgcn_s_setprio(3);
     if constexpr (FULL && GIVEN) load_tile_given64<SPLIT>(a, X, i0, lane, KP, c_aggs);
     else if constexpr (AHEAD)
-        load_tile_prog64_ahead<SPLIT>(a, X, i0, lane, KP, c_aggs, hdr_first, hdr_nb, ent_cur, x_first, ent_second, hdr_next_raw, hdr_first_next, hdr_nb_next, ent_next);
-    else if constexpr (PROG) load_tile_prog64<SPLIT>(a, X, i0, lane, KP, c_aggs, hdr_first, hdr_nb, ent_cur);
+        load_tile_prog64_ahead<SPLIT>(a, X, i0, lane, KP, c_aggs, hdr_first, hdr_nb, ent_cur, x_first, ent_second, hdr_next_raw, hdr_first_next, hdr_nb_next, tid_next, ent_next);
+    else if constexpr (PROG) {
+        load_tile_prog64<SPLIT>(a, X, i0, lane, KP, c_aggs, hdr_first, hdr_nb, ent_cur);
+        hdr_first_next = __builtin_amdgcn_readfirstlane(hdr_next_raw.x); hdr_nb_next = __builtin_amdgcn_readfirstlane(hdr_next_raw.y);
+        tid_next = __builtin_amdgcn_readfirstlane(hdr_next_raw.z);
+    }
     else if constexpr (FULL) load_tile_fast64<SPLIT, true>(a, X, ipt, i0, lane, KP, c_aggs, src_cur, w_cur);
     else {
         if (fast64) load_tile_fast64<SPLIT>(a, X, ipt, i0, lane, KP, c_aggs, src_cur, w_cur);
@@ -1415,7 +1421,6 @@
     float w_next = 0.0f;
     if constexpr (AHEAD) { }
     else if constexpr (PROG) {
-        hdr_first_next = __builtin_amdgcn_readfirstlane(hdr_next_raw.x); hdr_nb_next = __builtin_amdgcn_readfirstlane(hdr_next_raw.y);
         if (hdr_nb_next > 0) ent_next = prog_entry(a, hdr_first_next, lane);
     } else {
         ip_next = tile_rowptr_clamp(a, next_tile, lane, ip_next_raw);
@@ -1475,7 +1480,7 @@
         next_tile = __builtin_amdgcn_readfirstlane(next2_tile) + (third_round ? 2 * W_launch : 0) + a0.tile_base;
     } else next_tile = __builtin_amdgcn_readfirstlane(next2_tile) + a0.tile_base;
     ip_cur = ip_next; src_cur = src_next; w_cur = w_next;
-    hdr_first = hdr_first_next; hdr_nb = hdr_nb_next; ent_cur = ent_next;
+    hdr_first = hdr_first_next; hdr_nb = hdr_nb_next; tid = tid_next; ent_cur = ent_next;
   }
 }
 
diff --git a/gnn_tf_2.x_amd/csrc/gnn_graph.hip b/gnn_tf_2.x_amd/csrc/gnn_graph.hip
--- a/gnn_tf_2.x_amd/csrc/gnn_graph.hip
+++ b/gnn_tf_2.x_amd/csrc/gnn_graph.hip
@@ -94,7 +94,7 @@
     (void)hipFree(sh->src_indptr); (void)hipFree(sh->src_dst); (void)hipFree(sh->src_w);
     (void)hipFree(sh->arc_id); (void)hipFree(sh->arc_labels_orig);
     (void)hipFree(sh->full_indptr); (void)hipFree(sh->full_src); (void)hipFree(sh->full_w);
-    (void)hipFree(sh->gp_hdr); (void)hipFree(sh->gp_ent);
+    (void)hipFree(sh->gp_hdr); (void)hipFree(sh->gp_ent); (void)hipFree(sh->gp_slot[0]); (void)hipFree(sh->gp_slot[1]);
     delete sh;
 }
 
diff --git a/gnn_tf_2.x_amd/csrc/gnn_loop.hip b/gnn_tf_2.x_amd/csrc/gnn_loop.hip
--- a/gnn_tf_2.x_amd/csrc/gnn_loop.hip
+++ b/gnn_tf_2.x_amd/csrc/gnn_loop.hip
@@ -360,6 +360,15 @@
     l->gather_form = form;
     const int rc = gnn_loop_decide_form(l);
     if (used) *used = l->form.path == GNN_PATH_UNFUSED ? 0 : (l->form.program ? 2 : 1);
+    return rc;
+}
+
+extern "C" int gnn_loop_set_tile_schedule(gnn_loop *l, int kind, int *used)
+{
+    ARGCHK(l && kind >= 0 && kind <= 2, "kind must be 0 (library's choice), 1 (ascending tile order) or 2 (balanced tile order)");
+    l->tile_schedule = kind;
+    const int rc = gnn_loop_decide_form(l);
+    if (used) *used = l->form.path != GNN_PATH_UNFUSED && l->form.program ? l->form.schedule : 0;
     return rc;
 }
 
diff --git a/include/gnn_hip.h b/include/gnn_hip.h
--- a/include/gnn_hip.h
+++ b/include/gnn_hip.h
@@ -104,9 +104,12 @@
 int gnn_loop_set_persistent(gnn_loop *l, int enable, int *used);
 int gnn_loop_set_tile_form(gnn_loop *l, int form, int *used);
 int gnn_loop_set_gather_form(gnn_loop *l, int form, int *used);
+int gnn_loop_set_tile_schedule(gnn_loop *l, int kind, int *used);
 int gnn_gather_program_build(int64_t n_rows, const int32_t *indptr, const int32_t *adj_src, const float *adj_w, int32_t *hdr, int32_t *ent,
                              int64_t *n_batches);
 int gnn_graph_gather_program_info(const gnn_graph *g, int64_t *tiles, int64_t *batches, int64_t *bytes, float *build_ms);
+int gnn_tile_schedule_build(int64_t slots, const int64_t *cost, int64_t waves, int kind, int32_t *order);
+int gnn_graph_tile_schedule_info(const gnn_graph *g, int64_t *slots, int *kind, int64_t *body, int64_t *tail, float *build_ms);
 enum { GNN_FORM_PER_OP = 0, GNN_FORM_MLP_FWD = 1, GNN_FORM_WIDE = 2, GNN_FORM_CHAIN3 = 3, GNN_FORM_WGRAD_BF = 4, GNN_FORM_WGRAD_F32 = 5 };
 int gnn_train_forms(int n_layers, const int *dims, const int *acts, const float *rates, int64_t n_rows, int producer_dropout, int *out);
 int gnn_loop_train_forms(const gnn_loop *l, int net, int *out);
```

Measured after the change: 1.870 billion node-state-updates/s, median of 6. 3.1% higher.
